# fnysalehi/Surface-Irradiance-Estimation-from-Neural-Radiance-Fields

Measured on AMD Instinct MI355X. Metric: Mrays/s @1080p NeRF inference (Lego snapshot); PSNR vs reference, higher is better.
Workload: dtype f16; 1 GPU; Lego-shaped synthetic scene (HashGrid L8 F4 T2^19 b=2.0, density MLP 32-64-16, rgb MLP 32-64-64-16, aabb_scale 1), 1920x1080 pinhole camera fov_x 0.6911 rad, 8 orbit azimuths, 1 spp, render_mode Shade, min_transmittance 0.01; frames_in_flight=2

## Files before the change

__graft_entry__.py:

```python
import importlib
import os
import sys

ROOT = os.path.dirname(os.path.abspath(__file__))
PKG = "surface-irradiance-estimation-from-neural-radiance-fields_amd"
if ROOT not in sys.path:
    sys.path.insert(0, ROOT)


def _pkg(sub):
    return importlib.import_module(PKG + "." + sub)


def build():
    lib = _pkg("build").build()
    _pkg("build").build(legacy=True)
    _pkg("build").build(nocache=True)
    _pkg("build").build(netsec_v1=True)
    _pkg("build").build_pyngp()
    _pkg("build").build_main()
    sys.path.insert(0, os.path.join(ROOT, "oracle"))
    import oracle as orc

    orc.build()
    native = _pkg("native")
    L = native.load_library()
    missing = [s for s in native.EXPORTS if not hasattr(L, s)]
    if missing:
        raise RuntimeError(f"libngp_hip.so lacks symbols: {missing}")
    print(f"built {lib}; {L.ngp_version().decode()}")


def smoke():
    import numpy as np

    sys.path.insert(0, os.path.join(ROOT, "oracle"))
    import oracle as orc

    native, synthetic, scene = _pkg("native"), _pkg("synthetic"), _pkg("scene")
    sc = synthetic.make_scene(aabb_scale=1, seed=7, log2_hashmap_size=15)
    ctx = native.Context(0)
    ctx.set_model(sc)
    w, h = 96, 54
    mat = scene.orbit_camera(45.0)
    focal = scene.focal_from_fov_x(w, 0.6911)
    img, depth = ctx.render(native.make_camera(mat, w, h, focal), native.make_opts(), want_depth=True)
    st = ctx.render_stats()
    o = orc.Oracle()
    bf, _ = o.density_grid_to_bitfield(np.asarray(sc["density_grid"], np.float16).astype(np.float32), sc["max_cascade"])
    sc["density_grid_bitfield"] = bf
    m = o.make_model(sc)
    fb, db, ost = o.render_nerf(m, o.make_camera(mat, w, h, focal))
    ref = o.tonemap(o.accumulate(fb.reshape(-1, 4), np.zeros((w * h, 4), np.float32), 0)).reshape(h, w, 4)
    err = float(np.quantile(np.abs(img - ref), 0.9995))
    mse = float(((np.clip(img[..., :3], 0, 1) - np.clip(ref[..., :3], 0, 1)) ** 2).mean())
    psnr = 99.0 if mse == 0 else -10.0 * np.log10(mse)
    print(f"smoke: {w}x{h} hit={st['n_rays_hit']} (oracle {ost['n_rays_hit']}) samples={st['n_samples']} (oracle {ost['n_samples']}) "
          f"q99.95|d|={err:.2e} psnr={psnr:.1f} dB kernel={st['kernel_ms']:.3f} ms")
    assert st["n_rays_hit"] > 0 and psnr > 45.0 and err < 2e-2, "HIP render does not match the oracle"
    o.release(m)
    fsc = synthetic.make_scene(aabb_scale=1, seed=7, cfg=scene.frequency_network_config())
    fsc["density_grid_bitfield"] = bf
    ctx.set_model(fsc)
    rng = np.random.default_rng(0)
    pos = rng.uniform(0, 1, (777, 3)).astype(np.float32)
    d01 = rng.uniform(0, 1, (777, 3)).astype(np.float32)
    got = ctx.network(pos, d01).astype(np.float32)
    fm = o.make_model(fsc)
    want = o.network(fm, pos, d01).astype(np.float32)
    o.release(fm)
    ferr = float(np.abs(got - want).max())
    print(f"smoke: frequency.json network, 777 samples, max |d logit| = {ferr:.2e}")
    assert np.isfinite(got).all() and ferr < 6e-2, "the frequency.json network does not match the oracle"
    ctx.close()


if __name__ == "__main__":
    build()
    if "--smoke" in sys.argv:
        smoke()
```

surface-irradiance-estimation-from-neural-radiance-fields_amd/build.py:

```python
import os
import subprocess
import sys

HERE = os.path.dirname(os.path.abspath(__file__))
CSRC = os.path.join(HERE, "csrc")
LIB = os.path.join(HERE, "libngp_hip.so")
SOURCES = ["nerf_kernels.hip", "wide_kernels.hip", "mesh_kernels.hip", "train_kernels.hip", "mc_kernels.hip", "ngp_api.cpp", "ngp_model.cpp", "ngp_snapshot.cpp", "ngp_dataset.cpp", "ngp_render.cpp", "ngp_mesh.cpp", "ngp_train.cpp", "ngp_multi.cpp", "ngp_mc.cpp"]
FLAGS = ["--offload-arch=gfx950", "-O3", "-std=c++17", "-fPIC", "-shared", "-ffp-contract=off", "-fno-slp-vectorize", "-fvisibility=hidden", "-Wall", "-Wno-unused-function"]


def hipcc():
    for c in (os.environ.get("HIPCC"), "/opt/rocm/bin/hipcc", "hipcc"):
        if c and (os.path.isabs(c) and os.path.exists(c) or not os.path.isabs(c)):
            return c
    raise RuntimeError("hipcc not found")


LIB_LEGACY = os.path.join(HERE, "libngp_hip_legacy.so")
LIB_CELLSTATS = os.path.join(HERE, "libngp_hip_cellstats.so")
LIB_NOCACHE = os.path.join(HERE, "libngp_hip_nocache.so")
LIB_NETSEC_V1 = os.path.join(HERE, "libngp_hip_netsec_v1.so")


def needs_build(lib=LIB):
    if not os.path.exists(lib):
        return True
    t = os.path.getmtime(lib)
    for f in os.listdir(CSRC):
        if os.path.getmtime(os.path.join(CSRC, f)) > t:
            return True
    inc = os.path.join(HERE, "..", "include", "ngp_hip.h")
    return os.path.getmtime(inc) > t


def build(force=False, verbose=False, legacy=False, nocache=False, cellstats=False, netsec_v1=False):
    if legacy + nocache + cellstats + netsec_v1 > 1:
        raise ValueError("one variant at a time")
    lib = LIB_LEGACY if legacy else LIB_NOCACHE if nocache else LIB_CELLSTATS if cellstats else LIB_NETSEC_V1 if netsec_v1 else LIB
    if not force and not needs_build(lib):
        return lib
    srcs = [os.path.join(CSRC, s) for s in SOURCES if os.path.exists(os.path.join(CSRC, s))]
    tmp = "%s.%d.tmp" % (lib, os.getpid())
    cmd = [hipcc()] + FLAGS + (["-DNGP_TCNN_LEGACY_ENCODE"] if legacy else []) + (["-DNGP_NO_CELL_CACHE"] if nocache else []) + (["-DNGP_EXPERIMENT_CELL_CACHE_STATS"] if cellstats else []) + (["-DNGP_NETSEC_V1"] if netsec_v1 else []) + os.environ.get("NGP_BUILD_DEFINES", "").split() + ["-o", tmp] + srcs + ["-lz"]
    if verbose:
        print(" ".join(cmd))
    r = subprocess.run(cmd, capture_output=True, text=True)
    if r.returncode != 0:
        sys.stderr.write(r.stdout + r.stderr)
        if os.path.exists(tmp):
            os.remove(tmp)
        raise RuntimeError("hipcc failed")
    os.replace(tmp, lib)
    return lib


def pyngp_path():
    import sysconfig

    return os.path.join(HERE, "pyngp" + sysconfig.get_config_var("EXT_SUFFIX"))


def build_pyngp(force=False, verbose=False):
    import pybind11
    import sysconfig

    out = pyngp_path()
    srcs = [os.path.join(CSRC, "pyngp.cpp"), os.path.join(CSRC, "testbed_shim.h"), os.path.join(HERE, "..", "include", "ngp_hip.h")]
    if not force and os.path.exists(out) and all(os.path.getmtime(out) >= os.path.getmtime(s) for s in srcs):
        return out
    build()
    cmd = ["g++", "-O2", "-std=c++17", "-shared", "-fPIC", "-fvisibility=hidden", "-I", sysconfig.get_paths()["include"], "-I", pybind11.get_include(),
           srcs[0], "-o", out + ".%d.tmp" % os.getpid(), "-L", HERE, "-lngp_hip", "-Wl,-rpath,$ORIGIN"]
    if verbose:
        print(" ".join(cmd))
    r = subprocess.run(cmd, capture_output=True, text=True)
    if r.returncode != 0:
        sys.stderr.write(r.stdout + r.stderr)
        raise RuntimeError("building pyngp failed")
    os.replace(out + ".%d.tmp" % os.getpid(), out)
    return out


def main_path():
    return os.path.join(HERE, "ngp_hip_main")


def build_main(force=False, verbose=False):
    out = main_path()
    srcs = [os.path.join(CSRC, "ngp_main.cpp"), os.path.join(CSRC, "testbed_shim.h"), os.path.join(CSRC, "minijson.h"), os.path.join(HERE, "..", "include", "ngp_hip.h")]
    if not force and os.path.exists(out) and all(os.path.getmtime(out) >= os.path.getmtime(s) for s in srcs):
        return out
    build()
    cmd = ["g++", "-O2", "-std=c++17", "-Wall", srcs[0], "-o", out + ".%d.tmp" % os.getpid(), "-L", HERE, "-lngp_hip", "-lz", "-Wl,-rpath,$ORIGIN"]
    if verbose:
        print(" ".join(cmd))
    r = subprocess.run(cmd, capture_output=True, text=True)
    if r.returncode != 0:
        sys.stderr.write(r.stdout + r.stderr)
        raise RuntimeError("building ngp_hip_main failed")
    os.replace(out + ".%d.tmp" % os.getpid(), out)
    return out


def import_pyngp():
    import importlib.util

    path = build_pyngp()
    spec = importlib.util.spec_from_file_location("pyngp", path)
    mod = importlib.util.module_from_spec(spec)
    spec.loader.exec_module(mod)
    return mod


if __name__ == "__main__":
    print(build(force="--force" in sys.argv, verbose=True))
    print(build_pyngp(force="--force" in sys.argv, verbose=True))
```

surface-irradiance-estimation-from-neural-radiance-fields_amd/csrc/nerf_device.h:

```cpp
#pragma once

#include "ngp_kernels.h"
#include "cell_cache.h"

namespace ngp {

typedef _Float16 half_t;
typedef _Float16 half8 __attribute__((ext_vector_type(8)));
typedef float floatx4 __attribute__((ext_vector_type(4)));

struct f3 {
	float x, y, z;
};

#define NGP_DEV __device__ __forceinline__

#ifdef NGP_CENSUS
#define NGP_SECTION(name) asm volatile("; SECTION " name)
#else
#define NGP_SECTION(name)
#endif

NGP_DEV f3 mk3(float x, float y, float z) { return f3{x, y, z}; }
NGP_DEV f3 add3(f3 a, f3 b) { return mk3(a.x + b.x, a.y + b.y, a.z + b.z); }
NGP_DEV f3 sub3(f3 a, f3 b) { return mk3(a.x - b.x, a.y - b.y, a.z - b.z); }
NGP_DEV f3 mul3(f3 a, f3 b) { return mk3(a.x * b.x, a.y * b.y, a.z * b.z); }
NGP_DEV f3 div3(f3 a, f3 b) { return mk3(a.x / b.x, a.y / b.y, a.z / b.z); }
NGP_DEV f3 scale3(f3 a, float s) { return mk3(a.x * s, a.y * s, a.z * s); }
NGP_DEV f3 adds3(f3 a, float s) { return mk3(a.x + s, a.y + s, a.z + s); }
NGP_DEV float dot3(f3 a, f3 b) { return (a.x * b.x + a.y * b.y) + a.z * b.z; }
NGP_DEV f3 normalize3(f3 a) {
	float len = __builtin_sqrtf(dot3(a, a));
	return mk3(a.x / len, a.y / len, a.z / len);
}
NGP_DEV f3 m3_mulv(const float* m, f3 v) {
	f3 r = mk3(m[0] * v.x, m[1] * v.x, m[2] * v.x);
	r = add3(r, mk3(m[3] * v.y, m[4] * v.y, m[5] * v.y));
	r = add3(r, mk3(m[6] * v.z, m[7] * v.z, m[8] * v.z));
	return r;
}

NGP_DEV uint32_t laine_karras_permutation(uint32_t x, uint32_t seed) {
	x += seed;
	x ^= x * 0x6c50b47cu;
	x ^= x * 0xb82f1e52u;
	x ^= x * 0xc7afe638u;
	x ^= x * 0x8d22f6e6u;
	return x;
}
NGP_DEV uint32_t nested_uniform_scramble_base2(uint32_t x, uint32_t seed) {
	x = __builtin_bitreverse32(x);
	x = laine_karras_permutation(x, seed);
	return __builtin_bitreverse32(x);
}
NGP_DEV uint32_t hash_combine(uint32_t seed, uint32_t v) { return seed ^ (v + (seed << 6) + (seed >> 2)); }
NGP_DEV float ld_random_val_dim0(uint32_t index, uint32_t seed) {
	index = nested_uniform_scramble_base2(index, seed);
	uint32_t x = nested_uniform_scramble_base2(__builtin_bitreverse32(index), hash_combine(seed, 0u));
	return (float)x * 2.3283064365386963e-10f;
}

NGP_DEV float stepsize() { return 1.73205080757f / (float)NERF_STEPS; }
NGP_DEV float max_cone_stepsize() { return stepsize() * (float)(1u << (NERF_CASCADES - 1)) * (float)NERF_STEPS / (float)NERF_GRIDSIZE; }

NGP_DEV float div_const(float x, float d, float rc) {
	float q0 = x * rc;
	float r = __builtin_fmaf(-q0, d, x);
	return __builtin_fmaf(r, rc, q0);
}
NGP_DEV float div_stepsize(float x) { return div_const(x, stepsize(), 1.0f / stepsize()); }
NGP_DEV float div_max_cone_stepsize(float x) { return div_const(x, max_cone_stepsize(), 1.0f / max_cone_stepsize()); }

struct Stepping {
	float cone_angle, log1p_c, a, b, at, bt;
	float to_scale, from_scale;
};
NGP_DEV Stepping make_stepping(float cone_angle) {
	Stepping s;
	s.cone_angle = cone_angle;
	s.log1p_c = s.a = s.b = s.at = s.bt = s.to_scale = s.from_scale = 0.0f;
	if (cone_angle <= 1e-5f) return s;
	s.log1p_c = logf(1.0f + cone_angle);
	s.a = (logf(stepsize()) - logf(s.log1p_c)) / s.log1p_c;
	s.b = (logf(max_cone_stepsize()) - logf(s.log1p_c)) / s.log1p_c;
	s.at = expf(s.a * s.log1p_c);
	s.bt = expf(s.b * s.log1p_c);
	s.to_scale = 0.6931471805599453f / s.log1p_c;
	s.from_scale = s.log1p_c * 1.4426950408889634f;
	return s;
}
NGP_DEV float to_stepping_space(float t, const Stepping& s) {
	if (s.cone_angle <= 1e-5f) return div_stepsize(t);
	if (t <= s.at) return div_stepsize(t - s.at) + s.a;
#ifdef NGP_PRECISE_STEPPING
	else if (t <= s.bt) return logf(t) / s.log1p_c;
#else
	else if (t <= s.bt) return __builtin_amdgcn_logf(t) * s.to_scale;
#endif
	else return div_max_cone_stepsize(t - s.bt) + s.b;
}
NGP_DEV float from_stepping_space(float n, const Stepping& s) {
	if (s.cone_angle <= 1e-5f) return n * stepsize();
	if (n <= s.a) return (n - s.a) * stepsize() + s.at;
#ifdef NGP_PRECISE_STEPPING
	else if (n <= s.b) return expf(n * s.log1p_c);
#else
	else if (n <= s.b) return __builtin_amdgcn_exp2f(n * s.from_scale);
#endif
	else return (n - s.b) * max_cone_stepsize() + s.bt;
}
NGP_DEV float advance_n_steps(float t, const Stepping& s, float n) { return from_stepping_space(to_stepping_space(t, s) + n, s); }
NGP_DEV float calc_dt(float t, const Stepping& s) { return advance_n_steps(t, s, 1.0f) - t; }
NGP_DEV float to_stepping_space(float t, float cone_angle) { return to_stepping_space(t, make_stepping(cone_angle)); }
NGP_DEV float from_stepping_space(float n, float cone_angle) { return from_stepping_space(n, make_stepping(cone_angle)); }
NGP_DEV float advance_n_steps(float t, float cone_angle, float n) { return advance_n_steps(t, make_stepping(cone_angle), n); }
NGP_DEV float calc_dt(float t, float cone_angle) { return calc_dt(t, make_stepping(cone_angle)); }
NGP_DEV float warp_dt(float dt) {
	const float max_stepsize = stepsize() * (float)(1u << (NERF_CASCADES - 1));
	return div_const(dt - stepsize(), max_stepsize - stepsize(), 1.0f / (max_stepsize - stepsize()));
}
NGP_DEV float unwarp_dt(float dt) {
	float max_stepsize = stepsize() * (float)(1u << (NERF_CASCADES - 1));
	return dt * (max_stepsize - stepsize()) + stepsize();
}

NGP_DEV uint32_t expand_bits(uint32_t v) {
	v = (v * 0x00010001u) & 0xFF0000FFu;
	v = (v * 0x00000101u) & 0x0F00F00Fu;
	v = (v * 0x00000011u) & 0xC30C30C3u;
	v = (v * 0x00000005u) & 0x49249249u;
	return v;
}
NGP_DEV uint32_t morton3D(uint32_t x, uint32_t y, uint32_t z) { return expand_bits(x) | (expand_bits(y) << 1) | (expand_bits(z) << 2); }
NGP_DEV uint32_t morton3D_invert(uint32_t x) {
	x = x & 0x49249249u;
	x = (x | (x >> 2)) & 0xc30c30c3u;
	x = (x | (x >> 4)) & 0x0f00f00fu;
	x = (x | (x >> 8)) & 0xff0000ffu;
	x = (x | (x >> 16)) & 0x0000ffffu;
	return x;
}

NGP_DEV bool density_grid_occupied_at(f3 pos, const uint8_t* __restrict__ bitfield, uint32_t mip) {
	float mip_scale = __builtin_ldexpf(1.0f, -(int)mip);
	pos = adds3(scale3(adds3(pos, -0.5f), mip_scale), 0.5f);
	int ix = (int)(pos.x * (float)NERF_GRIDSIZE);
	int iy = (int)(pos.y * (float)NERF_GRIDSIZE);
	int iz = (int)(pos.z * (float)NERF_GRIDSIZE);
	if (ix < 0 || ix >= (int)NERF_GRIDSIZE || iy < 0 || iy >= (int)NERF_GRIDSIZE || iz < 0 || iz >= (int)NERF_GRIDSIZE) return false;
	uint32_t idx = morton3D((uint32_t)ix, (uint32_t)iy, (uint32_t)iz);
	return (bitfield[idx / 8 + (NERF_GRID_N_CELLS / 8) * mip] & (1u << (idx % 8))) != 0;
}

NGP_DEV bool density_grid_occupied_at_lds(f3 pos, const uint8_t* __restrict__ bitfield, const uint32_t* s_coarse, uint32_t mip) {
	float mip_scale = __builtin_ldexpf(1.0f, -(int)mip);
	pos = adds3(scale3(adds3(pos, -0.5f), mip_scale), 0.5f);
	int ix = (int)(pos.x * (float)NERF_GRIDSIZE);
	int iy = (int)(pos.y * (float)NERF_GRIDSIZE);
	int iz = (int)(pos.z * (float)NERF_GRIDSIZE);
	if (ix < 0 || ix >= (int)NERF_GRIDSIZE || iy < 0 || iy >= (int)NERF_GRIDSIZE || iz < 0 || iz >= (int)NERF_GRIDSIZE) return false;
	uint32_t idx = morton3D((uint32_t)ix, (uint32_t)iy, (uint32_t)iz);
	uint32_t block = idx >> 6;
	if (!((s_coarse[mip * COARSE_WORDS_PER_MIP + (block >> 5)] >> (block & 31u)) & 1u)) return false;
	return (bitfield[idx / 8 + (NERF_GRID_N_CELLS / 8) * mip] & (1u << (idx % 8))) != 0;
}

struct OccBlockCache {
	uint32_t key;
	uint2 bits;
};

NGP_DEV uint32_t empty_block_size_at(f3 pos, const uint8_t* __restrict__ bitfield, const uint32_t* s_coarse, const uint32_t* s_coarse16, uint32_t mip,
                                     OccBlockCache& cache) {
	float mip_scale = __builtin_ldexpf(1.0f, -(int)mip);
	pos = adds3(scale3(adds3(pos, -0.5f), mip_scale), 0.5f);
	int ix = (int)(pos.x * (float)NERF_GRIDSIZE);
	int iy = (int)(pos.y * (float)NERF_GRIDSIZE);
	int iz = (int)(pos.z * (float)NERF_GRIDSIZE);
	if (ix < 0 || ix >= (int)NERF_GRIDSIZE || iy < 0 || iy >= (int)NERF_GRIDSIZE || iz < 0 || iz >= (int)NERF_GRIDSIZE) return 1u;
	uint32_t idx = morton3D((uint32_t)ix, (uint32_t)iy, (uint32_t)iz);
	uint32_t b16 = idx >> 12;
	if (!((s_coarse16[mip * 16u + (b16 >> 5)] >> (b16 & 31u)) & 1u)) return 16u;
	uint32_t b4 = idx >> 6;
	if (!((s_coarse[mip * COARSE_WORDS_PER_MIP + (b4 >> 5)] >> (b4 & 31u)) & 1u)) return 4u;
	const uint32_t key = (mip << 26) | b4;
	if (cache.key != key) {
		cache.bits = *(const uint2*)(bitfield + (size_t)b4 * 8 + (size_t)(NERF_GRID_N_CELLS / 8) * mip);
		cache.key = key;
	}
	const uint32_t word = (idx & 32u) ? cache.bits.y : cache.bits.x;
	return ((word >> (idx & 31u)) & 1u) ? 0u : 1u;
}

struct OccBlock {
	uint32_t key;
	uint2 bits;
};
NGP_DEV uint32_t occupancy_state_at(f3 pos, const uint8_t* __restrict__ bitfield, const uint32_t* s_coarse, const uint32_t* s_coarse16, uint32_t mip, OccBlock& cache,
                                    uint32_t lds_mips = NERF_CASCADES, const uint32_t* __restrict__ g_coarse = nullptr) {
	float mip_scale = __builtin_ldexpf(1.0f, -(int)mip);
	pos = adds3(scale3(adds3(pos, -0.5f), mip_scale), 0.5f);
	const int ix = (int)(pos.x * (float)NERF_GRIDSIZE);
	const int iy = (int)(pos.y * (float)NERF_GRIDSIZE);
	const int iz = (int)(pos.z * (float)NERF_GRIDSIZE);
	if (((uint32_t)ix | (uint32_t)iy | (uint32_t)iz) >= NERF_GRIDSIZE) return 1u;
	const uint32_t x = (uint32_t)ix, y = (uint32_t)iy, z = (uint32_t)iz;
	const uint32_t key = (x >> 2) | ((y >> 2) << 5) | ((z >> 2) << 10) | (mip << 15);
	if (cache.key != key) {
		const uint32_t b4 = morton3D(x >> 2, y >> 2, z >> 2), b16 = b4 >> 6;
		if (!((s_coarse16[mip * 16u + (b16 >> 5)] >> (b16 & 31u)) & 1u)) return 16u;
		const uint32_t cw = mip < lds_mips ? s_coarse[mip * COARSE_WORDS_PER_MIP + (b4 >> 5)] : g_coarse[mip * COARSE_WORDS_PER_MIP + (b4 >> 5)];
		if (!((cw >> (b4 & 31u)) & 1u)) return 4u;
		cache.bits = *(const uint2*)(bitfield + (size_t)b4 * 8 + (size_t)(NERF_GRID_N_CELLS / 8) * mip);
		cache.key = key;
	}
	const uint32_t bit = (x & 1u) | ((y & 1u) << 1) | ((z & 1u) << 2) | ((x & 2u) << 2) | ((y & 2u) << 3) | ((z & 2u) << 4);
	const uint32_t word = (bit & 32u) ? cache.bits.y : cache.bits.x;
	return ((word >> (bit & 31u)) & 1u) ? 0u : 1u;
}

NGP_DEV uint32_t empty_block_summary_at(f3 pos, const uint32_t* s_coarse, const uint32_t* s_coarse16, uint32_t mip, uint32_t lds_mips = NERF_CASCADES,
                                        const uint32_t* __restrict__ g_coarse = nullptr) {
	float mip_scale = __builtin_ldexpf(1.0f, -(int)mip);
	pos = adds3(scale3(adds3(pos, -0.5f), mip_scale), 0.5f);
	const int ix = (int)(pos.x * (float)(NERF_GRIDSIZE / 4)), iy = (int)(pos.y * (float)(NERF_GRIDSIZE / 4)), iz = (int)(pos.z * (float)(NERF_GRIDSIZE / 4));
	if (((uint32_t)ix | (uint32_t)iy | (uint32_t)iz) >= NERF_GRIDSIZE / 4 || pos.x < 0.0f || pos.y < 0.0f || pos.z < 0.0f) return 0u;
	const uint32_t b4 = morton3D((uint32_t)ix, (uint32_t)iy, (uint32_t)iz), b16 = b4 >> 6;
	if (!((s_coarse16[mip * 16u + (b16 >> 5)] >> (b16 & 31u)) & 1u)) return 16u;
	const uint32_t cw = mip < lds_mips ? s_coarse[mip * COARSE_WORDS_PER_MIP + (b4 >> 5)] : g_coarse[mip * COARSE_WORDS_PER_MIP + (b4 >> 5)];
	return ((cw >> (b4 & 31u)) & 1u) ? 0u : 4u;
}

NGP_DEV float distance_to_next_voxel(f3 pos, f3 dir, f3 idir, float res, float inv_res) {
	f3 p = scale3(adds3(pos, -0.5f), res);
	float tx = (__builtin_floorf(p.x + 0.5f + 0.5f * __builtin_copysignf(1.0f, dir.x)) - p.x) * idir.x;
	float ty = (__builtin_floorf(p.y + 0.5f + 0.5f * __builtin_copysignf(1.0f, dir.y)) - p.y) * idir.y;
	float tz = (__builtin_floorf(p.z + 0.5f + 0.5f * __builtin_copysignf(1.0f, dir.z)) - p.z) * idir.z;
	float t = fminf(fminf(tx, ty), tz);
	return fmaxf(t * inv_res, 0.0f);
}
NGP_DEV float advance_to_next_voxel(float t, const Stepping& s, f3 pos, f3 dir, f3 idir, uint32_t mip, uint32_t block = 1u) {
	const int shift = block == 16u ? 4 : (block == 4u ? 2 : 0);
	float res = __builtin_ldexpf((float)NERF_GRIDSIZE, -(int)mip - shift);
	float t_target = t + distance_to_next_voxel(pos, dir, idir, res, __builtin_ldexpf(1.0f / (float)NERF_GRIDSIZE, (int)mip + shift));
	t = to_stepping_space(t, s);
	t_target = to_stepping_space(t_target, s);
	return from_stepping_space(t + __builtin_ceilf(fmaxf(t_target - t, 0.5f)), s);
}
NGP_DEV float advance_to_next_voxel(float t, float cone_angle, f3 pos, f3 dir, f3 idir, uint32_t mip, uint32_t block = 1u) {
	return advance_to_next_voxel(t, make_stepping(cone_angle), pos, dir, idir, mip, block);
}
NGP_DEV float grid_cube_entry(f3 pos, f3 idir, float h) {
	const float lo = 0.5f - h, hi = 0.5f + h;
	float tx0 = (lo - pos.x) * idir.x, tx1 = (hi - pos.x) * idir.x;
	float ty0 = (lo - pos.y) * idir.y, ty1 = (hi - pos.y) * idir.y;
	float tz0 = (lo - pos.z) * idir.z, tz1 = (hi - pos.z) * idir.z;
	float tmin = fmaxf(fmaxf(fminf(tx0, tx1), fminf(ty0, ty1)), fminf(tz0, tz1));
	float tmax = fminf(fminf(fmaxf(tx0, tx1), fmaxf(ty0, ty1)), fmaxf(tz0, tz1));
	tmin = fmaxf(tmin, 0.0f);
	return tmax >= tmin ? tmin : -1.0f;
}
NGP_DEV float advance_by_distance(float t, const Stepping& s, float distance) {
	float t_target = t + distance;
	t = to_stepping_space(t, s);
	t_target = to_stepping_space(t_target, s);
	return from_stepping_space(t + __builtin_ceilf(fmaxf(t_target - t, 0.5f)), s);
}
NGP_DEV float advance_by_distance(float t, float cone_angle, float distance) { return advance_by_distance(t, make_stepping(cone_angle), distance); }
NGP_DEV uint32_t mip_from_pos(f3 pos, uint32_t max_cascade) {
	int exponent;
	float maxval = fmaxf(fmaxf(__builtin_fabsf(pos.x - 0.5f), __builtin_fabsf(pos.y - 0.5f)), __builtin_fabsf(pos.z - 0.5f));
	(void)__builtin_frexpf(maxval, &exponent);
	int v = exponent + 1;
	v = v < 0 ? 0 : v;
	v = v > (int)max_cascade ? (int)max_cascade : v;
	return (uint32_t)v;
}

NGP_DEV bool raabb_contains(const ModelParams& M, f3 p) {
	if (!M.r2l_identity) p = m3_mulv(M.r2l, p);
	return p.x >= M.raabb_min[0] && p.x <= M.raabb_max[0] && p.y >= M.raabb_min[1] && p.y <= M.raabb_max[1] && p.z >= M.raabb_min[2] && p.z <= M.raabb_max[2];
}

template <bool CAPPED>
NGP_DEV float skip_empty_space(float t, const ModelParams& M, f3 o, f3 d, f3 idir) {
	const float cone_angle = M.cone_angle;
	uint32_t i = 1;
	while (!CAPPED || i < 200) {
		f3 pos = add3(o, scale3(d, t));
		if (t >= MAX_DEPTH || !raabb_contains(M, pos)) return MAX_DEPTH;
		uint32_t mip = mip_from_pos(pos, NERF_CASCADES - 1);
		mip = mip > M.max_cascade ? M.max_cascade : mip;
		if (density_grid_occupied_at(pos, M.bitfield, mip)) return t;
		while (mip < M.max_cascade && !density_grid_occupied_at(pos, M.bitfield, mip + 1)) ++mip;
		t = advance_to_next_voxel(t, cone_angle, pos, d, idir, mip);
		++i;
	}
	return MAX_DEPTH;
}

NGP_DEV float aabb_ray_entry(const float* bmin, const float* bmax, f3 pos, f3 dir) {
	const float FMAX = 3.402823466e+38f;
	float tmin = (bmin[0] - pos.x) / dir.x;
	float tmax = (bmax[0] - pos.x) / dir.x;
	if (tmin > tmax) { float s = tmin; tmin = tmax; tmax = s; }
	float tymin = (bmin[1] - pos.y) / dir.y;
	float tymax = (bmax[1] - pos.y) / dir.y;
	if (tymin > tymax) { float s = tymin; tymin = tymax; tymax = s; }
	if (tmin > tymax || tymin > tmax) return FMAX;
	if (tymin > tmin) tmin = tymin;
	if (tymax < tmax) tmax = tymax;
	float tzmin = (bmin[2] - pos.z) / dir.z;
	float tzmax = (bmax[2] - pos.z) / dir.z;
	if (tzmin > tzmax) { float s = tzmin; tzmin = tzmax; tzmax = s; }
	if (tmin > tzmax || tzmin > tmax) return FMAX;
	if (tzmin > tmin) tmin = tzmin;
	return tmin;
}

struct RayState {
	f3 o, d;
	float t;
	uint32_t idx;
	uint32_t out;
	bool alive;
};

NGP_DEV void opencv_lens_distortion_delta(const float* q, float u, float v, float* du, float* dv) {
	const float k1 = q[0], k2 = q[1], p1 = q[2], p2 = q[3];
	const float u2 = u * u, uv = u * v, v2 = v * v, r2 = u2 + v2;
	const float radial = k1 * r2 + k2 * r2 * r2;
	*du = u * radial + 2.0f * p1 * uv + p2 * (r2 + 2.0f * u2);
	*dv = v * radial + 2.0f * p2 * uv + p1 * (r2 + 2.0f * v2);
}
NGP_DEV void opencv_fisheye_lens_distortion_delta(const float* q, float u, float v, float* du, float* dv) {
	const float k1 = q[0], k2 = q[1], k3 = q[2], k4 = q[3];
	const float r = __builtin_sqrtf(u * u + v * v);
	if (r > (float)2.220446049250313e-16) {
		const float theta = atanf(r);
		const float theta2 = theta * theta, theta4 = theta2 * theta2, theta6 = theta4 * theta2, theta8 = theta4 * theta4;
		const float thetad = theta * (1.0f + k1 * theta2 + k2 * theta4 + k3 * theta6 + k4 * theta8);
		*du = u * thetad / r - u;
		*dv = v * thetad / r - v;
	} else {
		*du = 0.0f;
		*dv = 0.0f;
	}
}
template <bool FISHEYE>
NGP_DEV void iterative_lens_undistortion(const float* q, float* u, float* v) {
	auto delta = [&](float a, float b, float* da, float* db) {
		if (FISHEYE) opencv_fisheye_lens_distortion_delta(q, a, b, da, db);
		else opencv_lens_distortion_delta(q, a, b, da, db);
	};
	const float x0 = *u, y0 = *v;
	float x = x0, y = y0;
	for (uint32_t i = 0; i < 100u; ++i) {
		const float step0 = fmaxf(1.1920929e-07f, __builtin_fabsf(1e-6f * x));
		const float step1 = fmaxf(1.1920929e-07f, __builtin_fabsf(1e-6f * y));
		float dx0, dx1, b0, b1, f0, f1, c0, c1, g0, g1;
		delta(x, y, &dx0, &dx1);
		delta(x - step0, y, &b0, &b1);
		delta(x + step0, y, &f0, &f1);
		delta(x, y - step1, &c0, &c1);
		delta(x, y + step1, &g0, &g1);
		const float j00 = 1.0f + (f0 - b0) / (2.0f * step0), j10 = (g0 - c0) / (2.0f * step1);
		const float j01 = (f1 - b1) / (2.0f * step0), j11 = 1.0f + (g1 - c1) / (2.0f * step1);
		const float rx = x + dx0 - x0, ry = y + dx1 - y0;
		const float det = j00 * j11 - j10 * j01;
		const float sx = (j11 * rx - j10 * ry) / det, sy = (-j01 * rx + j00 * ry) / det;
		x -= sx;
		y -= sy;
		if (sx * sx + sy * sy < 1e-10f) break;
	}
	*u = x;
	*v = y;
}
__device__ __attribute__((noinline)) void lens_direction_general(int lens_mode, const float* lens_params, float u, float v, float sx, float sy, float* out) {
	const float PI = 3.14159265358979323846f;
	f3 dir;
	if (lens_mode == 3) {
		float theta = (v - 0.5f) * PI, phi = (u - 0.5f) * PI * 2.0f;
// ... 107 lines not shown
	const float phi = atan2f(dy, dx);
	const float cyl_x = theta / PI, cyl_y = phi / (2.0f * PI) + 0.5f;
	const float fx = cyl_y * (float)(res_x - 1), fy = cyl_x * (float)(res_y - 1);
	const int tx = (int)fx, ty = (int)fy;
	const float wx = fx - (float)tx, wy = fy - (float)ty;
	auto read_val = [&](int px, int py) {
		if (px < 0) px += res_x;
		else if (px >= res_x) px -= res_x;
		py = py > res_y - 1 ? res_y - 1 : py;
		py = py < 0 ? 0 : py;
		return envmap[px + (size_t)py * res_x];
	};
	const float4 v00 = read_val(tx, ty), v10 = read_val(tx + 1, ty), v01 = read_val(tx, ty + 1), v11 = read_val(tx + 1, ty + 1);
	const float w00 = (1 - wx) * (1 - wy), w10 = wx * (1 - wy), w01 = (1 - wx) * wy, w11 = wx * wy;
	out4[0] = ((w00 * v00.x + w10 * v10.x) + w01 * v01.x) + w11 * v11.x;
	out4[1] = ((w00 * v00.y + w10 * v10.y) + w01 * v01.y) + w11 * v11.y;
	out4[2] = ((w00 * v00.z + w10 * v10.z) + w01 * v01.z) + w11 * v11.z;
	out4[3] = ((w00 * v00.w + w10 * v10.w) + w01 * v01.w) + w11 * v11.w;
}

template <bool PLAIN = false>
NGP_DEV void init_ray(const ModelParams& M, const CameraParams& C, uint32_t x, uint32_t y, RayState& r) {
	r.idx = x + (uint32_t)C.width * y;
	r.out = r.idx;
	float u = ((float)x + C.pixel_offset[0]) / (float)C.width;
	float v = ((float)y + C.pixel_offset[1]) / (float)C.height;
	f3 dir;
	if (PLAIN) dir = mk3((u - C.screen_center[0]) * (float)C.width / C.focal[0], (v - C.screen_center[1]) * (float)C.height / C.focal[1], 1.0f);
	else lens_direction(C, u, v, dir);
	f3 origin;
	if (PLAIN || !C.moving) {
		dir = m3_mulv(C.m, dir);
		origin = mk3(C.m[9], C.m[10], C.m[11]);
		if (!PLAIN && C.aperture_size != 0.0f) {
			float o3[3] = {origin.x, origin.y, origin.z}, d3[3] = {dir.x, dir.y, dir.z}, cm[6];
			for (int i = 0; i < 6; ++i) cm[i] = C.m[i];
			apply_aperture(cm, C.aperture_size, C.focus_z, C.spp, (uint32_t)(int)(u * (float)C.width) * 19349663u + (uint32_t)(int)(v * (float)C.height) * 96925573u, o3, d3);
			origin = mk3(o3[0], o3[1], o3[2]);
			dir = mk3(d3[0], d3[1], d3[2]);
		}
	} else {
		float cam[12], m0[12], m1[12], rs[4];
		for (int i = 0; i < 12; ++i) { m0[i] = C.m[i]; m1[i] = C.m1[i]; }
		for (int i = 0; i < 4; ++i) rs[i] = C.rolling_shutter[i];
		camera_at_pixel(m0, m1, rs, u, v, ld_random_val_dim0(C.spp, r.idx * 72239731u), cam);
		dir = m3_mulv(cam, dir);
		origin = mk3(cam[9], cam[10], cam[11]);
		if (C.aperture_size != 0.0f) {
			float o3[3] = {origin.x, origin.y, origin.z}, d3[3] = {dir.x, dir.y, dir.z};
			apply_aperture(cam, C.aperture_size, C.focus_z, C.spp, (uint32_t)(int)(u * (float)C.width) * 19349663u + (uint32_t)(int)(v * (float)C.height) * 96925573u, o3, d3);
			origin = mk3(o3[0], o3[1], o3[2]);
			dir = mk3(d3[0], d3[1], d3[2]);
		}
	}
	origin = add3(origin, scale3(dir, C.near_distance));
	r.o = origin;
	r.d = mk3(0.f, 0.f, 0.f);
	r.t = 0.f;
	r.alive = false;
	if (dir.x == 0.0f && dir.y == 0.0f && dir.z == 0.0f) return;
	dir = normalize3(dir);
	r.d = dir;
	float t = fmaxf(aabb_ray_entry(M.raabb_min, M.raabb_max, m3_mulv(M.r2l, origin), m3_mulv(M.r2l, dir)), 0.0f) + 1e-6f;
	if (!raabb_contains(M, add3(origin, scale3(dir, t)))) return;
	r.t = t;
	r.alive = true;
}

NGP_DEV void advance_pos(const ModelParams& M, const CameraParams& C, RayState& r) {
	if (!r.alive) return;
	f3 idir = mk3(1.0f / r.d.x, 1.0f / r.d.y, 1.0f / r.d.z);
	float t = advance_n_steps(r.t, M.cone_angle, ld_random_val_dim0(C.spp, r.idx * 786433u));
	t = skip_empty_space<false>(t, M, r.o, r.d, idir);
	if (t >= MAX_DEPTH) r.alive = false;
	else r.t = t;
}

struct CornerSet {
	uint32_t index[8];
};

struct CellPos {
	uint32_t gx, gy, gz;
	float wx, wy, wz;
};
NGP_DEV CellPos level_cell(const LevelInfo& L, float x, float y, float z) {
	float fx = __builtin_fmaf(L.scale, x, 0.5f), fy = __builtin_fmaf(L.scale, y, 0.5f), fz = __builtin_fmaf(L.scale, z, 0.5f);
	float flx = __builtin_floorf(fx), fly = __builtin_floorf(fy), flz = __builtin_floorf(fz);
	CellPos c;
	c.gx = (uint32_t)(int)flx; c.gy = (uint32_t)(int)fly; c.gz = (uint32_t)(int)flz;
	c.wx = fx - flx; c.wy = fy - fly; c.wz = fz - flz;
	return c;
}
NGP_DEV CellPos level_cell_in_cube(const LevelInfo& L, float x, float y, float z) {
	const float fx = __builtin_fmaf(L.scale, x, 0.5f), fy = __builtin_fmaf(L.scale, y, 0.5f), fz = __builtin_fmaf(L.scale, z, 0.5f);
	CellPos c;
	c.gx = (uint32_t)fx; c.gy = (uint32_t)fy; c.gz = (uint32_t)fz;
	c.wx = __builtin_amdgcn_fractf(fx); c.wy = __builtin_amdgcn_fractf(fy); c.wz = __builtin_amdgcn_fractf(fz);
	return c;
}
NGP_DEV void corner_weights(const CellPos& p, float* weight) {
	float wx0 = 1.0f - p.wx, wy0 = 1.0f - p.wy, wz0 = 1.0f - p.wz;
#pragma unroll
	for (int c = 0; c < 8; ++c) {
		int bx = c & 1, by = (c >> 1) & 1, bz = (c >> 2) & 1;
		weight[c] = ((bx ? p.wx : wx0) * (by ? p.wy : wy0)) * (bz ? p.wz : wz0);
	}
}
NGP_DEV bool level_in_xor_range(const LevelInfo& L, const CellPos& p) {
	uint32_t m = p.gx > p.gy ? p.gx : p.gy;
	m = m > p.gz ? m : p.gz;
	return m <= L.coord_max && !L.xor_disabled;
}
NGP_DEV bool unit_cube_in_xor_range(const LevelInfo* lv) {
	bool ok = true;
	for (int l = 0; l < N_LEVELS; ++l) ok = ok && !lv[l].xor_disabled && (uint32_t)__builtin_fmaf(lv[l].scale, 1.0f, 0.5f) <= lv[l].coord_max;
	return ok;
}
NGP_DEV bool in_unit_cube(float x, float y, float z) { return fminf(fminf(x, y), z) >= 0.0f && fmaxf(fmaxf(x, y), z) <= 1.0f; }

NGP_DEV void level_corners(const LevelInfo& L, const CellPos& p, CornerSet& cs) {
	uint32_t ix[2], iy[2], iz[2];
	if (L.hashed) {
		ix[0] = p.gx;               ix[1] = p.gx + 1u;
		iy[0] = p.gy * 2654435761u; iy[1] = (p.gy + 1u) * 2654435761u;
		iz[0] = p.gz * 805459861u;  iz[1] = (p.gz + 1u) * 805459861u;
	} else {
		uint32_t r2 = L.res * L.res;
		ix[0] = p.gx;         ix[1] = p.gx + 1u;
		iy[0] = p.gy * L.res; iy[1] = (p.gy + 1u) * L.res;
		iz[0] = p.gz * r2;    iz[1] = (p.gz + 1u) * r2;
	}
#pragma unroll
	for (int c = 0; c < 8; ++c) {
		int bx = c & 1, by = (c >> 1) & 1, bz = (c >> 2) & 1;
		uint32_t idx = L.hashed ? (ix[bx] ^ iy[by] ^ iz[bz]) : (ix[bx] + iy[by] + iz[bz]);
		idx = L.mask ? (idx & L.mask) : (idx % L.size);
		cs.index[c] = (L.offset + idx) * 8u;
	}
}

NGP_DEV void level_corners_xor(const LevelInfo& L, const CellPos& p, CornerSet& cs) {
	uint32_t ix[2], iy[2], iz[2];
	ix[0] = p.gx << 3;        ix[1] = ix[0] + 8u;
	iy[0] = p.gy * L.mul_y8;  iy[1] = iy[0] + L.mul_y8;
	iz[0] = p.gz * L.mul_z8;  iz[1] = iz[0] + L.mul_z8;
#pragma unroll
	for (int c = 0; c < 8; ++c) {
		int bx = c & 1, by = (c >> 1) & 1, bz = (c >> 2) & 1;
		cs.index[c] = ((ix[bx] ^ iy[by] ^ iz[bz]) & L.mask8) | L.base8;
	}
}

typedef unsigned int u32x2 __attribute__((ext_vector_type(2)));
typedef __amdgpu_buffer_rsrc_t GridRsrc;
NGP_DEV GridRsrc make_grid_rsrc(const void* table, uint32_t bytes) { return __builtin_amdgcn_make_buffer_rsrc(const_cast<void*>(table), (short)0, (int)bytes, 0x00020000); }
NGP_DEV uint2 gather8(GridRsrc r, uint32_t offset) {
	const u32x2 v = __builtin_amdgcn_raw_buffer_load_b64(r, (int)offset, 0, 0);
	return make_uint2(v.x, v.y);
}

typedef _Float16 half2_t __attribute__((ext_vector_type(2)));
NGP_DEV half_t to_half_rn(float v) {
	asm("" : "+v"(v));
	return (half_t)v;
}
struct FeatureAcc {
	half2_t f01, f23;
};
NGP_DEV float product_lo(float w, uint32_t packed) {
	float p;
	asm("v_fma_mix_f32 %0, %1, %2, 0 op_sel_hi:[0,1,0]" : "=v"(p) : "v"(w), "v"(packed));
	return p;
}
NGP_DEV float product_hi(float w, uint32_t packed) {
	float p;
	asm("v_fma_mix_f32 %0, %1, %2, 0 op_sel:[0,1,0] op_sel_hi:[0,1,0]" : "=v"(p) : "v"(w), "v"(packed));
	return p;
}
NGP_DEV void accumulate_corner(uint2 v, float w, FeatureAcc& r) {
#ifndef NGP_TCNN_LEGACY_ENCODE
	const half2_t wh = {(half_t)w, (half_t)w};
	const uint32_t wv = __builtin_bit_cast(uint32_t, wh);
	uint32_t a01 = __builtin_bit_cast(uint32_t, r.f01), a23 = __builtin_bit_cast(uint32_t, r.f23);
	asm("v_pk_fma_f16 %0, %1, %2, %0" : "+v"(a01) : "v"(wv), "v"(v.x));
	asm("v_pk_fma_f16 %0, %1, %2, %0" : "+v"(a23) : "v"(wv), "v"(v.y));
	r.f01 = __builtin_bit_cast(half2_t, a01);
	r.f23 = __builtin_bit_cast(half2_t, a23);
#else
	half2_t a, b;
	a[0] = (half_t)product_lo(w, v.x);
	a[1] = (half_t)product_hi(w, v.x);
	b[0] = (half_t)product_lo(w, v.y);
	b[1] = (half_t)product_hi(w, v.y);
	r.f01 = r.f01 + a;
	r.f23 = r.f23 + b;
#endif
}
NGP_DEV void accumulate_corner_pair(uint2 v0, uint2 v1, half2_t w01, FeatureAcc& r) {
	const uint32_t wv = __builtin_bit_cast(uint32_t, w01);
	uint32_t a01 = __builtin_bit_cast(uint32_t, r.f01), a23 = __builtin_bit_cast(uint32_t, r.f23);
	asm("v_pk_fma_f16 %0, %1, %2, %0 op_sel:[0,0,0] op_sel_hi:[0,1,1]" : "+v"(a01) : "v"(wv), "v"(v0.x));
	asm("v_pk_fma_f16 %0, %1, %2, %0 op_sel:[0,0,0] op_sel_hi:[0,1,1]" : "+v"(a23) : "v"(wv), "v"(v0.y));
	asm("v_pk_fma_f16 %0, %1, %2, %0 op_sel:[1,0,0] op_sel_hi:[1,1,1]" : "+v"(a01) : "v"(wv), "v"(v1.x));
	asm("v_pk_fma_f16 %0, %1, %2, %0 op_sel:[1,0,0] op_sel_hi:[1,1,1]" : "+v"(a23) : "v"(wv), "v"(v1.y));
	r.f01 = __builtin_bit_cast(half2_t, a01);
	r.f23 = __builtin_bit_cast(half2_t, a23);
}
NGP_DEV void store_features(const FeatureAcc& lo, const FeatureAcc& hi, half8& out) {
	out[0] = lo.f01[0]; out[1] = lo.f01[1]; out[2] = lo.f23[0]; out[3] = lo.f23[1];
	out[4] = hi.f01[0]; out[5] = hi.f01[1]; out[6] = hi.f23[0]; out[7] = hi.f23[1];
}

struct EncodeInFlight {
	uint2 v[16];
	float wx[2], wy[2], wz[2];
	uint32_t cell;
};
NGP_DEV void encode_issue(GridRsrc grid, GridRsrc xgrid, const LevelInfo* lv, int h, float x, float y, float z, EncodeInFlight& e) {
	const LevelInfo& L0 = lv[h];
	const LevelInfo& L1 = lv[h + 4];
	const CellPos p0 = level_cell(L0, x, y, z), p1 = level_cell(L1, x, y, z);
	CornerSet c0, c1;
	if (__all((int)level_in_xor_range(L0, p0) & (int)level_in_xor_range(L1, p1))) {
		level_corners_xor(L0, p0, c0);
		level_corners_xor(L1, p1, c1);
#pragma unroll
		for (int c = 0; c < 8; ++c) e.v[c] = gather8(xgrid, c0.index[c]);
#pragma unroll
		for (int c = 0; c < 8; ++c) e.v[8 + c] = gather8(xgrid, c1.index[c]);
#if defined(NGP_EXPERIMENT_EXTRA_GATHERS)
#pragma unroll
		for (int c = 0; c < NGP_EXPERIMENT_EXTRA_GATHERS; ++c) {
			const uint2 d = gather8(xgrid, c & 1 ? c1.index[c & 7] : c0.index[c & 7]);
			asm volatile("" ::"v"(d.x), "v"(d.y));
		}
#endif
	} else {
		level_corners(L0, p0, c0);
		level_corners(L1, p1, c1);
#pragma unroll
		for (int c = 0; c < 8; ++c) e.v[c] = gather8(grid, c0.index[c]);
#pragma unroll
		for (int c = 0; c < 8; ++c) e.v[8 + c] = gather8(grid, c1.index[c]);
	}
	e.wx[0] = p0.wx; e.wy[0] = p0.wy; e.wz[0] = p0.wz;
	e.wx[1] = p1.wx; e.wy[1] = p1.wy; e.wz[1] = p1.wz;
}
NGP_DEV half8 encode_finish(const EncodeInFlight& e) {
	NGP_SECTION("encode_finish");
	FeatureAcc acc[2] = {{{0, 0}, {0, 0}}, {{0, 0}, {0, 0}}};
#pragma unroll
	for (int l = 0; l < 2; ++l) {
		CellPos p;
		p.gx = p.gy = p.gz = 0;
		p.wx = e.wx[l]; p.wy = e.wy[l]; p.wz = e.wz[l];
		float w[8];
		corner_weights(p, w);
#if defined(NGP_TCNN_LEGACY_ENCODE) || defined(NGP_NETSEC_V1)
#pragma unroll
		for (int c = 0; c < 8; ++c) accumulate_corner(e.v[8 * l + c], w[c], acc[l]);
#else
#pragma unroll
		for (int c = 0; c < 8; c += 2) {
			const half2_t w01 = {to_half_rn(w[c]), to_half_rn(w[c + 1])};
			accumulate_corner_pair(e.v[8 * l + c], e.v[8 * l + c + 1], w01, acc[l]);
		}
#endif
	}
	half8 out;
	store_features(acc[0], acc[1], out);
	NGP_SECTION("network");
	return out;
}
constexpr int CELL_CACHE_SETS = 8;
struct CellCache {
	uint4 line[CELL_CACHE_LEVELS][CELL_CACHE_SETS][4];
	uint32_t tag[CELL_CACHE_LEVELS][CELL_CACHE_SETS];
};
NGP_DEV void cell_cache_clear(CellCache* caches, int n_waves, int thread, int n_threads) {
	for (int i = thread; i < n_waves * CELL_CACHE_LEVELS * CELL_CACHE_SETS; i += n_threads)
		caches[i / (CELL_CACHE_LEVELS * CELL_CACHE_SETS)].tag[i / CELL_CACHE_SETS % CELL_CACHE_LEVELS][i % CELL_CACHE_SETS] = CELL_TAG_NONE;
}
NGP_DEV void encode_issue_cached(GridRsrc grid, GridRsrc xgrid, const LevelInfo* lv, int h, float x, float y, float z, EncodeInFlight& e, CellCache& cc, bool in_cube) {
	NGP_SECTION("issue.cells");
	const LevelInfo& L0 = lv[h];
	const LevelInfo& L1 = lv[h + 4];
#ifdef NGP_NETSEC_V1
	CellPos p0 = level_cell(L0, x, y, z), p1 = level_cell(L1, x, y, z);
	in_cube = __all((int)level_in_xor_range(L0, p0) & (int)level_in_xor_range(L1, p1));
#else
	CellPos p0, p1;
#endif
	CornerSet c0, c1;
	e.cell = CELL_TAG_NONE;
	if (in_cube) {
#ifndef NGP_NETSEC_V1
		p0 = level_cell_in_cube(L0, x, y, z);
		p1 = level_cell_in_cube(L1, x, y, z);
#endif
		NGP_SECTION("issue.fine");
		level_corners_xor(L1, p1, c1);
#pragma unroll
		for (int c = 0; c < 8; ++c) e.v[8 + c] = gather8(xgrid, c1.index[c]);
		NGP_SECTION("issue.tag_lines");
		const bool cacheable = cell_cacheable(p0.gx, p0.gy, p0.gz);
		const uint32_t tag = cell_tag(p0.gx, p0.gy, p0.gz), set = cell_set(tag, CELL_CACHE_SETS);
		const bool hit = __hip_atomic_load(&cc.tag[h][set], __ATOMIC_RELAXED, __HIP_MEMORY_SCOPE_WAVEFRONT) == tag && cacheable;
#pragma unroll
		for (int q = 0; q < 4; ++q) {
			const uint4 d = cc.line[h][set][q];
			e.v[2 * q] = make_uint2(d.x, d.y);
			e.v[2 * q + 1] = make_uint2(d.z, d.w);
// ... 397 lines not shown
```

surface-irradiance-estimation-from-neural-radiance-fields_amd/csrc/nerf_kernels.hip:

```cpp
#include "render_common.h"
#include "pcg32.h"

namespace ngp {

constexpr int BLOCK = 256;

#if defined(NGP_NO_CELL_CACHE) || defined(NGP_EXPERIMENT_CELL_CACHE_STATS)
constexpr bool CELL_CACHE_BUILT = false;
#else
constexpr bool CELL_CACHE_BUILT = true;
#endif
struct FusedGeneric {
	static constexpr bool probe = false, unit = false, outside = true, plain = false, normals = false, cell_cache = false;
	static constexpr int prof = 0, mips = (int)NERF_CASCADES, rgb_mid = 1;
};
struct FusedUnit : FusedGeneric { static constexpr bool unit = true, cell_cache = CELL_CACHE_BUILT; static constexpr int mips = 1; };
struct FusedUnitPlain : FusedUnit { static constexpr bool plain = true; };
struct FusedC5 : FusedGeneric { static constexpr bool outside = false; static constexpr int mips = 4; };
struct FusedC5Plain : FusedC5 { static constexpr bool plain = true; };
struct FusedMid0 : FusedGeneric { static constexpr int rgb_mid = 0; };
struct FusedMid2 : FusedGeneric { static constexpr int rgb_mid = 2; };
struct FusedLinRgb : FusedGeneric { static constexpr int rgb_mid = -1; };
struct FusedLin : FusedGeneric { static constexpr int rgb_mid = -2; };
struct FusedNormals : FusedGeneric { static constexpr bool normals = true; };
struct FusedProf : FusedGeneric { static constexpr int prof = 1; };
struct FusedUnitPlainProf : FusedUnitPlain { static constexpr int prof = 1; };
struct FusedUnitPlainProf2 : FusedUnitPlain { static constexpr int prof = 2; };
struct FusedProbe : FusedGeneric { static constexpr bool probe = true; };

template <class V>
NGP_DEV void fused_body(const ModelParams& M, const CameraParams& C, const FrameParams& F, const ProbeParams& P) {
	constexpr bool PROBE = V::probe, UNIT = V::unit, OUTSIDE = V::outside, PLAIN = V::plain, NORMALS = V::normals, CELL_CACHE = V::cell_cache;
	constexpr int PROF = V::prof, MIPS = V::mips, RGB_MID = V::rgb_mid;
	const uint32_t max_cascade = UNIT ? 0u : M.max_cascade;
	const float cone_angle = UNIT ? 0.0f : M.cone_angle;
	const Stepping stepping = make_stepping(cone_angle);
	__shared__ uint4 s_w[n_frags_for(RGB_MID) * 64];
	__shared__ LevelInfo s_lv[N_LEVELS];
	__shared__ uint32_t s_coarse[MIPS * COARSE_WORDS_PER_MIP];
	__shared__ uint32_t s_coarse16[(UNIT ? 1 : (int)NERF_CASCADES) * 16];
	__shared__ uint2 s_sh[BLOCK * 4];
	constexpr int SLOTS = 64;
	__shared__ float4 s_samp[BLOCK / 64 * SLOTS];
	__shared__ uint2 s_res[BLOCK / 64 * SLOTS];
	__shared__ float4 s_nrm[NORMALS ? BLOCK / 64 * SLOTS : 1];
	__shared__ CellCache s_cells[CELL_CACHE ? BLOCK / 64 : 1];
#ifdef NGP_EXPERIMENT_CELL_CACHE_STATS
	__shared__ uint32_t s_cst[BLOCK / 64][CELL_CACHE_LEVELS][4 + 8 + 16];
	for (int i = threadIdx.x; i < BLOCK / 64 * CELL_CACHE_LEVELS * 28; i += BLOCK) (&s_cst[0][0][0])[i] = CELL_TAG_NONE;
	unsigned long long cst_n = 0, cst_hit[3] = {0, 0, 0};
#endif
	__shared__ uint32_t s_xstate, s_xcount, s_active;
	constexpr uint32_t XRAYS = 16;
	__shared__ float s_xray[XRAYS * 16];
	if (threadIdx.x == 0) {
		s_xstate = 0u;
		s_xcount = 0u;
		s_active = BLOCK / 64;
	}
	unsigned long long t_entry = 0, rt_entry = 0;
	if (PROF) { t_entry = stamp(); rt_entry = realtime(); }
	for (int i = threadIdx.x; i < n_frags_for(RGB_MID) * 64; i += BLOCK) s_w[i] = M.wfrags[i];
	if (threadIdx.x < N_LEVELS) s_lv[threadIdx.x] = M.levels[threadIdx.x];
	for (uint32_t i = threadIdx.x; i < (max_cascade + 1 < (uint32_t)MIPS ? max_cascade + 1 : (uint32_t)MIPS) * COARSE_WORDS_PER_MIP; i += BLOCK) s_coarse[i] = M.coarse[i];
	if (threadIdx.x < (UNIT ? 1 : (int)NERF_CASCADES) * 16) s_coarse16[threadIdx.x] = M.coarse[NERF_CASCADES * COARSE_WORDS_PER_MIP + threadIdx.x];
	if (CELL_CACHE) cell_cache_clear(s_cells, BLOCK / 64, threadIdx.x, BLOCK);
	__syncthreads();

	const int lane = threadIdx.x & 63;
	const int c = lane & 15;
	if (lane == 0 && (threadIdx.x >> 6) == 0) atomicMax(&F.results[4], ~realtime());
	const GridRsrc t_grid = make_grid_rsrc(M.grid, M.grid_bytes), t_xgrid = make_grid_rsrc(M.xgrid, M.xgrid_bytes);
	const bool cube_in_xor_range = CELL_CACHE && unit_cube_in_xor_range(M.levels);
	(void)cube_in_xor_range;
	const float* cam_last = (!PLAIN && C.moving) ? C.m1 : C.m;
	const f3 cam_fwd = mk3(cam_last[6], cam_last[7], cam_last[8]);
	const f3 bg_linear = (PROBE || !F.direct) ? mk3(0.f, 0.f, 0.f)
	                     : F.color_space == 1 ? mk3(F.background[0], F.background[1], F.background[2])
	                                          : mk3(srgb_to_linear(F.background[0]), srgb_to_linear(F.background[1]), srgb_to_linear(F.background[2]));
	const float4 empty_pixel = (!PROBE && F.direct) ? tonemap_pixel(F, bg_linear, 0.f, 0.f, 0.f, 0.f) : make_float4(0.f, 0.f, 0.f, 0.f);
	const f3 cam_pos = mk3(cam_last[9], cam_last[10], cam_last[11]);
	const f3 amin = mk3(M.aabb_min[0], M.aabb_min[1], M.aabb_min[2]);
	const f3 adiag = mk3(M.aabb_diag[0], M.aabb_diag[1], M.aabb_diag[2]);

	RayState ray;
	ray.alive = false;
	ray.o = ray.d = mk3(0.f, 0.f, 0.f);
	ray.t = 0.f;
	ray.idx = 0;
	ray.out = 0;
	f3 idir = mk3(0.f, 0.f, 0.f);
	Accum acc = {0.f, 0.f, 0.f, 0.f, 0.f, 0.f};
	uint32_t step = 1;
	uint32_t skip_i = 1;
	float t_max = 0.f;
	bool counted = false;
	uint32_t n_pend = 0, sl_lo = 0, sl_hi = 0;
	bool left_box = false;
	uint32_t n_slots = 0;
	const int wave_base = threadIdx.x & ~63;
	OccBlock occ_cache;
	occ_cache.key = 0xffffffffu;
	occ_cache.bits = make_uint2(0u, 0u);
	bool finished = false;
	bool idle = false;
	const uint32_t my_wave = threadIdx.x >> 6;

	bool exhausted = false;
	uint32_t qsel = (uint32_t)__builtin_amdgcn_s_getreg(20 | (0 << 6) | (3 << 11)) & 7u;
	int stall = 0;
	uint32_t n_alive_init = 0, n_hit = 0, n_samples = 0;
	unsigned long long p_skip[3] = {0, 0, 0};
	unsigned long long pt[4] = {0, 0, 0, 0}, p_iters = 0, p_passes = 0, p_rounds = 0, p_lane_steps = 0, t0 = 0, t1 = 0;

	unsigned long long rt_start = 0;
	if (PROF && F.prof) {
		rt_start = realtime();
		if (lane == 0) atomicMax(&F.prof[8], ~rt_start);
	}
	int tr_slot = -1;
	uint32_t tr_it = 0, tr_info0 = 0, tr_info1 = 0, tr_march = 0;
	uint32_t tr_net[7] = {0, 0, 0, 0, 0, 0, 0};
	unsigned long long tr_t[5] = {0, 0, 0, 0, 0};
	auto trace_emit = [&](int upto) {
		if (!PROF || tr_slot < 0) return;
		if (tr_it < F.trace_cap_iters && lane == 0) {
			uint32_t* r = F.trace + 16 + F.trace_cap_waves * 16u + ((size_t)tr_slot * F.trace_cap_iters + tr_it) * 16u;
			r[0] = (uint32_t)tr_t[0];
			for (int k = 1; k < 5; ++k) r[k] = (uint32_t)(tr_t[k <= upto ? k : upto] - tr_t[0]);
			r[5] = tr_info0;
			r[6] = tr_info1;
			r[7] = tr_march;
			for (int k = 0; k < 7; ++k) r[8 + k] = upto >= 3 ? tr_net[k] : 0u;
		}
		++tr_it;
	};
	for (;;) {
		if (PROF) { t0 = stamp(); tr_t[0] = t0; tr_info0 = tr_info1 = tr_march = 0; for (int k = 0; k < 7; ++k) tr_net[k] = 0; }
		unsigned long long dead_mask = __ballot(!ray.alive);
		int n_dead = __popcll(dead_mask);
		if ((exhausted || n_dead >= F.tune[0]) && __any(finished)) {
			bool hit = false;
			if (finished) {
				hit = shade_ray<PROBE, PLAIN, NORMALS>(F, P, bg_linear, ray.out, acc, step - 1u, ray.d);
				finished = false;
			}
			n_hit += (uint32_t)__popcll(__ballot(hit));
			if (PROF) tr_info1 |= 4u << 24;
		}
		if (!exhausted && n_dead >= (F.tune[0] > 16 ? F.tune[0] : 16)) {
			const uint32_t want = (uint32_t)n_dead >> 4, n_strips = F.n_local_tiles * 4u;
			uint32_t first = 0, limit = n_strips;
			if (!PROBE && F.xqueue) {
				for (int tries = 0; tries < 8; ++tries) {
					const uint32_t lo = (uint32_t)(((unsigned long long)n_strips * qsel) >> 3), hi = (uint32_t)(((unsigned long long)n_strips * (qsel + 1u)) >> 3);
					uint32_t off = 0;
					if (lane == 0) off = atomicAdd(F.xqueue + qsel, want);
					off = __builtin_amdgcn_readfirstlane(off);
					first = lo + off;
					limit = hi;
					if (off < hi - lo) break;
					first = limit = n_strips;
					qsel = (qsel + 1u) & 7u;
				}
			} else {
				if (lane == 0) first = atomicAdd(F.queue, want);
				first = __builtin_amdgcn_readfirstlane(first);
			}
			if (first >= limit) {
				exhausted = true;
			} else {
				const uint32_t got = limit - first < want ? limit - first : want;
				if (PROF && F.trace && tr_slot == -1) {
					uint32_t n = 0;
					if (lane == 0) n = atomicAdd(F.trace, 1u);
					n = __builtin_amdgcn_readfirstlane(n);
					tr_slot = (n % F.trace_stride == 0u && n / F.trace_stride < F.trace_cap_waves) ? (int)(n / F.trace_stride) : -2;
					if (tr_slot >= 0 && lane == 0) {
						uint32_t* hd = F.trace + 16 + (size_t)tr_slot * 16u;
						hd[0] = (uint32_t)__builtin_amdgcn_s_getreg(4 | (0 << 6) | (31 << 11));
						hd[1] = (uint32_t)__builtin_amdgcn_s_getreg(20 | (0 << 6) | (3 << 11)) & 7u;
						hd[2] = blockIdx.x;
						hd[3] = threadIdx.x >> 6;
						hd[5] = (uint32_t)rt_entry; hd[6] = (uint32_t)(rt_entry >> 32);
						hd[9] = (uint32_t)t_entry; hd[10] = (uint32_t)tr_t[0];
						hd[11] = n;
					}
				}
				if (PROF) tr_info1 |= 8u << 24;
				const uint32_t r = lanes_below(dead_mask);
				const uint32_t strip = first + (r >> 4);
				const bool take = !ray.alive && r < got * 16u;
				const uint32_t tile_local = strip >> 2, s4 = strip & 3u, i16 = r & 15u;
				const uint32_t slot = ((s4 >> 1) * 4u + (i16 >> 2)) * 8u + (s4 & 1u) * 4u + (i16 & 3u);
				const uint32_t tile = F.shard_index + F.shard_count * tile_local;
				bool fresh = false;
				if (PROBE) {
					uint32_t q = tile * 64u + slot;
					if (take && q < P.n_rays) {
						init_probe_ray(P, q, ray, t_max);
						fresh = ray.alive;
					}
				} else if (take) {
					uint32_t x = (tile % F.tiles_x) * 8u + (slot & 7u);
					uint32_t y = (tile / F.tiles_x) * 8u + (slot >> 3);
					if (x < (uint32_t)C.width && y < (uint32_t)C.height) {
						init_ray<PLAIN>(M, C, x, y, ray);
						if (F.packed) ray.out = tile_local * 64u + slot;
						if (PLAIN || !F.envmap) {
							if (F.direct) {
								F.frame_buffer[ray.out] = empty_pixel;
								F.depth_buffer[ray.out] = MAX_DEPTH;
							} else if (F.depth_buffer[ray.out] < 0.01f) {
								F.depth_buffer[ray.out] = MAX_DEPTH;
							}
						} else {
							const bool valid = ray.d.x != 0.0f || ray.d.y != 0.0f || ray.d.z != 0.0f;
							float env[4] = {0.f, 0.f, 0.f, 0.f};
							if (valid) {
								float d3[3] = {ray.d.x, ray.d.y, ray.d.z};
								read_envmap(F.envmap, F.env_w, F.env_h, d3, env);
							}
							if (F.direct) {
								F.frame_buffer[ray.out] = valid ? tonemap_pixel(F, bg_linear, env[0], env[1], env[2], env[3]) : empty_pixel;
								F.depth_buffer[ray.out] = MAX_DEPTH;
							} else {
								if (valid) F.frame_buffer[ray.out] = make_float4(env[0], env[1], env[2], env[3]);
								if (F.depth_buffer[ray.out] < 0.01f) F.depth_buffer[ray.out] = MAX_DEPTH;
							}
						}
						if (ray.alive) {
							ray.t = advance_n_steps(ray.t, stepping, ld_random_val_dim0(C.spp, ray.idx * 786433u));
							fresh = true;
						}
					}
				}
				if (fresh) {
					{
						union { half_t h[16]; uint2 u[4]; } sh;
						sh4_all((ray.d.x + 1.0f) * 0.5f, (ray.d.y + 1.0f) * 0.5f, (ray.d.z + 1.0f) * 0.5f, sh.h);
#pragma unroll
						for (int q = 0; q < 4; ++q) s_sh[threadIdx.x * 4 + q] = sh.u[q];
					}
					idir = mk3(1.0f / ray.d.x, 1.0f / ray.d.y, 1.0f / ray.d.z);
					acc = Accum{0.f, 0.f, 0.f, 0.f, 0.f, 0.f};
					step = 1;
					skip_i = 1;
					counted = PROBE;
				}
				if (PROBE) n_alive_init += (uint32_t)__popcll(__ballot(fresh));
			}
		}

		if (!PROBE && F.tune[7] && n_slots == 0u) {
			const uint32_t st = __hip_atomic_load(&s_xstate, __ATOMIC_RELAXED, __HIP_MEMORY_SCOPE_WORKGROUP);
			const unsigned long long live_mask = __ballot(ray.alive);
			if ((st & 0xf00u) == 0x100u && __popcll(live_mask) >= 16) {
				const uint32_t to = st & 0xffu;
				uint32_t won = 0;
				if (lane == 0) won = atomicCAS(&s_xstate, st, 0x200u | to) == st ? 1u : 0u;
				won = __builtin_amdgcn_readfirstlane(won);
				if (won) {
					const uint32_t rank = lanes_below(live_mask);
					if (ray.alive && (rank & 1u) && (rank >> 1) < XRAYS) {
						const uint32_t k = rank >> 1;
						float* x = s_xray + k * 16u;
						x[0] = ray.o.x; x[1] = ray.o.y; x[2] = ray.o.z;
						x[3] = ray.d.x; x[4] = ray.d.y; x[5] = ray.d.z;
						x[6] = ray.t;
						x[7] = __uint_as_float(ray.out);
						x[8] = acc.r; x[9] = acc.g; x[10] = acc.b; x[11] = acc.a; x[12] = acc.depth; x[13] = acc.max_weight;
						x[14] = __uint_as_float(step | (counted ? 0x80000000u : 0u));
						x[15] = __uint_as_float(ray.idx);
#pragma unroll
						for (int q = 0; q < 4; ++q) s_sh[(to * 64u + k) * 4u + q] = s_sh[threadIdx.x * 4 + q];
						ray.alive = false;
					}
					if (lane == 0) {
						atomicAdd(&s_active, 1u);
						const uint32_t n_out = (uint32_t)__popcll(live_mask) >> 1;
						s_xcount = n_out < XRAYS ? n_out : XRAYS;
						__hip_atomic_store(&s_xstate, 0x300u | to, __ATOMIC_RELEASE, __HIP_MEMORY_SCOPE_WORKGROUP);
					}
				}
			}
		}
		if (PROF) { t1 = stamp(); pt[0] += t1 - t0; t0 = t1; tr_t[1] = t1; }
		const int n_live = __popcll(__ballot(ray.alive));
		const int k_fit = n_live <= 8 ? 8 : (n_live <= 10 ? 6 : (n_live <= 12 ? 5 : (n_live <= 16 ? 4 : (n_live <= 21 ? 3 : 2))));
		const int k_max = PROBE ? 1 : (n_live > SLOTS / 2 ? F.tune[4] : (k_fit < F.tune[5] ? k_fit : F.tune[5]));
		const int max_it = F.tune[1] > k_max ? F.tune[1] : k_max;
		bool blocked = false;
		for (int k = 0; k < max_it; ++k) {
			NGP_SECTION("march");
			const bool marching = ray.alive && !left_box && !blocked && (int)n_pend < k_max;
			if (!__any(marching) || n_slots >= (uint32_t)SLOTS) break;
			if (PROF) { const uint32_t nm = (uint32_t)__popcll(__ballot(marching)); ++p_rounds; p_lane_steps += (unsigned long long)nm; tr_march += 1u + (nm << 8); }
			const f3 pos = add3(ray.o, scale3(ray.d, ray.t));
			bool out = ray.t >= MAX_DEPTH || !raabb_contains(M, pos);
			if (PROBE && skip_i >= 200) out = true;
			if (PROBE && ray.t >= t_max) out = true;
			const bool inside = marching && !out;
			uint32_t mip = 0, empty = 1u;
			if (inside) {
				if (!UNIT) {
					mip = mip_from_pos(pos, NERF_CASCADES - 1);
					mip = mip > max_cascade ? max_cascade : mip;
				}
				empty = occupancy_state_at(pos, M.bitfield, s_coarse, s_coarse16, mip, occ_cache, MIPS, M.coarse);
			}
			const bool emit = inside && empty == 0u;
			const bool skip = inside && empty != 0u;
			float e_dt = 0.f;
			f3 e_w = mk3(0.f, 0.f, 0.f);
			if (emit) {
				e_dt = calc_dt(ray.t, stepping);
				e_w = sub3(pos, amin);
				if (M.diag_pow2) e_w = mul3(e_w, mk3(M.aabb_inv_diag[0], M.aabb_inv_diag[1], M.aabb_inv_diag[2]));
				else e_w = div3(e_w, adiag);
			}
			bool ends = marching && out;
			if (skip) {
				if (!UNIT) {
					if (PROBE || !F.tune[6]) {
						while (mip < max_cascade) {
							uint32_t e = occupancy_state_at(pos, M.bitfield, s_coarse, s_coarse16, mip + 1, occ_cache, MIPS, M.coarse);
							if (e == 0u) break;
							++mip;
							empty = e;
						}
					} else {
						uint32_t best_mip = mip, best_empty = empty;
						for (uint32_t m = mip + 1u; m <= max_cascade; ++m) {
							const uint32_t e = empty_block_summary_at(pos, s_coarse, s_coarse16, m, MIPS, M.coarse);
							if (e == 0u) break;
							if ((e << m) >= (best_empty << best_mip)) { best_mip = m; best_empty = e; }
						}
						mip = best_mip;
						empty = best_empty;
					}
				}
				if (PROF) p_skip[empty == 16u ? 2 : (empty == 4u ? 1 : 0)] += 1ull;
				const float grid_half = 0.5f * (float)(1u << max_cascade);
				const bool outside = OUTSIDE && !PROBE && empty == 1u && mip == max_cascade &&
				                     fmaxf(fmaxf(__builtin_fabsf(pos.x - 0.5f), __builtin_fabsf(pos.y - 0.5f)), __builtin_fabsf(pos.z - 0.5f)) > grid_half;
				const float to_grid = outside ? grid_cube_entry(pos, idir, grid_half) : 0.0f;
				if (outside && to_grid < 0.0f) {
					ends = true;
				} else if (outside && to_grid > 0.0f) {
					ray.t = advance_by_distance(ray.t, stepping, to_grid);
				} else {
					ray.t = advance_to_next_voxel(ray.t, stepping, pos, ray.d, idir, mip, (PROBE || !F.tune[6]) ? 1u : empty);
				}
				++skip_i;
			}
			if (ends) {
				if (n_pend == 0) {
					ray.alive = false;
					finished = true;
				} else {
					left_box = true;
				}
			}
			const unsigned long long emit_mask = __ballot(emit);
			if (emit_mask) {
				const uint32_t slot = n_slots + lanes_below(emit_mask);
				bool newly_counted = false;
				if (emit) {
					newly_counted = !counted;
					counted = true;
					if (slot < (uint32_t)SLOTS) {
						s_samp[wave_base + slot] = make_float4(e_w.x, e_w.y, e_w.z, warp_dt(e_dt));
						s_res[wave_base + slot].x = (uint32_t)lane;
						if (n_pend < 4u) sl_lo |= slot << (8u * n_pend);
						else sl_hi |= slot << (8u * (n_pend - 4u));
						++n_pend;
						ray.t = ray.t + e_dt;
						skip_i = 1;
					} else {
						blocked = true;
					}
				}
				n_alive_init += (uint32_t)__popcll(__ballot(newly_counted));
				n_slots += (uint32_t)__popcll(emit_mask);
				n_slots = n_slots > (uint32_t)SLOTS ? (uint32_t)SLOTS : n_slots;
			}
		}
		NGP_SECTION("other");
		const bool can_march = __any(ray.alive && !left_box && !blocked && (int)n_pend < k_max);
		if (PROF) {
			t1 = stamp(); pt[1] += t1 - t0; t0 = t1; ++p_iters; tr_t[2] = t1;
			tr_info0 = n_slots | ((uint32_t)stall << 24);
			tr_info1 |= (uint32_t)__popcll(__ballot(ray.alive)) | ((uint32_t)__popcll(__ballot(ray.alive && !left_box && n_pend == 0)) << 8) | ((uint32_t)k_max << 16) |
			            ((exhausted ? 1u : 0u) << 24);
		}
		if (n_slots == 0) {
			trace_emit(2);
			if (exhausted && !__any(ray.alive) && !__any(finished)) {
				if (PROBE || !F.tune[7]) break;
				if (!idle) {
					idle = true;
					if (lane == 0) atomicSub(&s_active, 1u);
				}
				bool got = false;
				for (;;) {
					uint32_t st = 0, act = 0;
					if (lane == 0) {
						st = __hip_atomic_load(&s_xstate, __ATOMIC_ACQUIRE, __HIP_MEMORY_SCOPE_WORKGROUP);
						act = __hip_atomic_load(&s_active, __ATOMIC_RELAXED, __HIP_MEMORY_SCOPE_WORKGROUP);
					}
					st = __builtin_amdgcn_readfirstlane(st);
					act = __builtin_amdgcn_readfirstlane(act);
					if (st == (0x300u | my_wave)) {
						got = true;
						break;
					}
					if (act == 0u) break;
					if (st == 0u && lane == 0) atomicCAS(&s_xstate, 0u, 0x100u | my_wave);
					__builtin_amdgcn_s_sleep(32);
				}
				if (!got) break;
				const uint32_t n_in = s_xcount;
				if ((uint32_t)lane < n_in) {
					const float* x = s_xray + (uint32_t)lane * 16u;
					ray.o = mk3(x[0], x[1], x[2]);
					ray.d = mk3(x[3], x[4], x[5]);
					ray.t = x[6];
					ray.out = __float_as_uint(x[7]);
					acc = Accum{x[8], x[9], x[10], x[11], x[12], x[13]};
					const uint32_t sw = __float_as_uint(x[14]);
					step = sw & 0x7fffffffu;
					counted = (sw >> 31) != 0u;
					ray.idx = __float_as_uint(x[15]);
					idir = mk3(1.0f / ray.d.x, 1.0f / ray.d.y, 1.0f / ray.d.z);
					ray.alive = true;
					finished = false;
					left_box = false;
					skip_i = 1;
					n_pend = 0;
					sl_lo = sl_hi = 0;
					occ_cache.key = 0xffffffffu;
				}
				idle = false;
				if (lane == 0) __hip_atomic_store(&s_xstate, 0u, __ATOMIC_RELEASE, __HIP_MEMORY_SCOPE_WORKGROUP);
			}
			continue;
		}
		if ((int)n_slots < F.tune[2] && can_march && stall < F.tune[3]) {
			++stall;
			trace_emit(2);
			continue;
		}
		stall = 0;

		NGP_SECTION("network");
		const int n_pass = (int)((n_slots + 15u) >> 4);
		const int hq = lane >> 4;
		auto sample_of = [&](int p, float& sx, float& sy, float& sz, Sh4& shq) {
			NGP_SECTION("sample_of");
			const float4 a = s_samp[wave_base + 16 * p + c];
			const uint32_t owner = s_res[wave_base + 16 * p + c].x;
			sx = a.x; sy = a.y; sz = a.z;
			union { uint2 u; half_t h[4]; } cv;
#ifdef NGP_NETSEC_V1
			cv.u = s_sh[(wave_base + (int)owner) * 4 + hq];
#else
			cv.u = s_sh[(wave_base + (int)(owner & 63u)) * 4 + hq];
#endif
#pragma unroll
			for (int j = 0; j < 4; ++j) shq.v[j] = cv.h[j];
			NGP_SECTION("network");
		};
		auto deliver = [&](int p, const MlpOut& mo) {
			NGP_SECTION("deliver");
			union { half_t h[4]; uint2 u; } o;
			o.h[0] = mo.rgb[0]; o.h[1] = mo.rgb[1]; o.h[2] = mo.rgb[2]; o.h[3] = mo.sigma;
			if (lane < 16) s_res[wave_base + 16 * p + lane] = o.u;
			NGP_SECTION("network");
		};
		int p = 0;
		if (NORMALS) {
			for (; p < n_pass; ++p) {
				float ax, ay, az;
				Sh4 sha;
				sample_of(p, ax, ay, az, sha);
				EncodeInFlight e;
				encode_issue(t_grid, t_xgrid, s_lv, hq, ax, ay, az, e);
				const half8 enc = encode_finish(e);
				DensityGrad dg = density_gradient_pass(s_w, M.wfrags, lane, e, enc, s_lv[hq].scale, s_lv[hq + 4].scale, M.density_linear != 0);
#pragma unroll
				for (int k = 0; k < 3; ++k) {
					dg.g[k] += __shfl_xor(dg.g[k], 16, 64);
					dg.g[k] += __shfl_xor(dg.g[k], 32, 64);
				}
				if (lane < 16) s_nrm[wave_base + 16 * p + lane] = make_float4(dg.g[0] * (1.0f / 128.0f), dg.g[1] * (1.0f / 128.0f), dg.g[2] * (1.0f / 128.0f), (float)dg.sigma);
			}
		}
		bool round_in_cube = true;
#ifndef NGP_NETSEC_V1
		if constexpr (CELL_CACHE) {
			NGP_SECTION("round_range");
			const float4 a = s_samp[wave_base + lane];
			round_in_cube = cube_in_xor_range && !__any((uint32_t)lane < n_slots && !in_unit_cube(a.x, a.y, a.z));
			NGP_SECTION("network");
		}
#endif
		auto issue = [&](float sx, float sy, float sz, EncodeInFlight& e) {
			if constexpr (CELL_CACHE) encode_issue_cached(t_grid, t_xgrid, s_lv, hq, sx, sy, sz, e, s_cells[my_wave], round_in_cube);
			else encode_issue(t_grid, t_xgrid, s_lv, hq, sx, sy, sz, e);
#ifdef NGP_EXPERIMENT_CELL_CACHE_STATS
			const CellPos p = level_cell(s_lv[hq], sx, sy, sz);
			e.cell = CELL_TAG_NONE;
			if (level_in_xor_range(s_lv[hq], p) && cell_cacheable(p.gx, p.gy, p.gz)) {
				const uint32_t tag = cell_tag(p.gx, p.gy, p.gz);
				e.cell = tag;
				++cst_n;
				for (int k = 0; k < 3; ++k) {
					const bool hit = s_cst[my_wave][hq][(4 << k) - 4 + cell_set(tag, 4u << k)] == tag;
					cst_hit[k] += hit ? 1u : 0u;
					e.cell |= hit ? 0u : 1u << (24 + k);
				}
			}
#endif
		};
		auto keep = [&](const EncodeInFlight& e) {
			if constexpr (CELL_CACHE) cell_cache_fill(s_cells[my_wave], hq, e);
#ifdef NGP_EXPERIMENT_CELL_CACHE_STATS
			if (e.cell != CELL_TAG_NONE)
				for (int k = 0; k < 3; ++k)
					if (e.cell >> (24 + k) & 1u) s_cst[my_wave][hq][(4 << k) - 4 + cell_set(e.cell & 0xFFFFFFu, 4u << k)] = e.cell & 0xFFFFFFu;
#endif
		};
		unsigned long long u0 = 0, u1 = 0;
		auto lap = [&](int k, bool drain_gathers) {
			if (drain_gathers) asm volatile("s_waitcnt vmcnt(0)" ::: "memory");
			else if (k == 5) asm volatile("s_waitcnt lgkmcnt(0)" ::: "memory");
			u1 = stamp();
			tr_net[k] += (uint32_t)(u1 - u0);
			u0 = u1;
		};
		if (PROF >= 2) u0 = stamp();
		for (; p + 1 < n_pass; p += 2) {
			float ax, ay, az, bx, by, bz;
			Sh4 sha, shb;
			sample_of(p, ax, ay, az, sha);
			sample_of(p + 1, bx, by, bz, shb);
			EncodeInFlight ea, eb;
			issue(ax, ay, az, ea);
			issue(bx, by, bz, eb);
			if (PROF >= 2) { lap(0, false); if (CELL_CACHE) lap(5, false); lap(1, true); }
			half8 enca = encode_finish(ea);
			half8 encb = encode_finish(eb);
			if (PROF >= 2) lap(2, false);
			keep(ea);
			keep(eb);
			if (PROF >= 2 && CELL_CACHE) lap(6, false);
#ifdef NGP_NETSEC_V1
			MlpOut moa = mlp_pass<RGB_MID>(s_w, lane, enca, sha);
			MlpOut mob = mlp_pass<RGB_MID>(s_w, lane, encb, shb);
#else
			MlpOut moa, mob;
			mlp_pass2<RGB_MID>(s_w, lane, enca, sha, encb, shb, moa, mob);
#endif
			if (PROF >= 2) lap(3, false);
			deliver(p, moa);
			deliver(p + 1, mob);
			if (PROF >= 2) lap(4, false);
		}
		if (p < n_pass) {
			float ax, ay, az;
			Sh4 sha;
			sample_of(p, ax, ay, az, sha);
			EncodeInFlight e1;
			issue(ax, ay, az, e1);
			if (PROF >= 2) { lap(0, false); if (CELL_CACHE) lap(5, false); lap(1, true); }
			half8 enc = encode_finish(e1);
			if (PROF >= 2) lap(2, false);
			keep(e1);
			if (PROF >= 2 && CELL_CACHE) lap(6, false);
			MlpOut mo = mlp_pass<RGB_MID>(s_w, lane, enc, sha);
			if (PROF >= 2) lap(3, false);
			deliver(p, mo);
			if (PROF >= 2) lap(4, false);
		}

		if (PROF) { t1 = stamp(); pt[2] += t1 - t0; t0 = t1; p_passes += (unsigned long long)n_pass; tr_t[3] = t1; tr_info0 |= (n_slots << 8) | ((uint32_t)n_pass << 16); }
		for (uint32_t k = 0;; ++k) {
			NGP_SECTION("composite");
			const bool have = k < n_pend && ray.alive;
			if (!__any(have)) break;
			if (have) {
				const uint32_t slot = ((k < 4u ? sl_lo >> (8u * k) : sl_hi >> (8u * (k - 4u))) & 0xffu);
				const float4 a = s_samp[wave_base + slot];
				union { uint2 u; half_t h[4]; } o;
				o.u = s_res[wave_base + slot];
				float gx = 0.f, gy = 0.f, gz = 0.f;
				if (NORMALS) {
					const float4 g = s_nrm[wave_base + slot];
					gx = g.x; gy = g.y; gz = g.z;
					o.h[3] = (half_t)g.w;
				}
				const f3 pos = add3(amin, mul3(mk3(a.x, a.y, a.z), adiag));
				const float sdepth = PROBE ? dot3(ray.d, sub3(pos, ray.o))
				                          : dot3(cam_fwd, sub3(pos, cam_pos));
				float T = 1.0f - acc.a;
				float dt = unwarp_dt(a.w);
				float alpha = 1.0f - fast_exp(-network_to_density((float)o.h[3], M.density_act) * dt);
				float weight = alpha * T;
				float cr = network_to_rgb((float)o.h[0], M.rgb_act), cg = network_to_rgb((float)o.h[1], M.rgb_act), cb = network_to_rgb((float)o.h[2], M.rgb_act);
				if (!PROBE && F.render_mode > 1) {
					if (NORMALS) {
						const float dd = network_to_density_derivative((float)o.h[3], M.density_act);
						const f3 nrm = normalize3(mk3(-dd * gx, -dd * gy, -dd * gz));
						cr = nrm.x; cg = nrm.y; cb = nrm.z;
					} else if (F.render_mode == 2) {
						cr = cg = cb = alpha;
					} else if (F.render_mode == 3) {
						cr = (pos.x - 0.5f) / 2.0f + 0.5f; cg = (pos.y - 0.5f) / 2.0f + 0.5f; cb = (pos.z - 0.5f) / 2.0f + 0.5f;
					} else {
						cr = cg = cb = dot3(cam_fwd, sub3(pos, ray.o)) * F.depth_scale;
					}
				}
				acc.r += cr * weight;
				acc.g += cg * weight;
				acc.b += cb * weight;
				acc.a += weight;
				if (weight > acc.max_weight) {
					acc.max_weight = weight;
					acc.depth = sdepth;
				}
				++step;
				if (acc.a > (1.0f - F.min_transmittance)) {
					acc.r /= acc.a; acc.g /= acc.a; acc.b /= acc.a; acc.a /= acc.a;
					ray.alive = false;
					finished = true;
				} else if (step >= MARCH_ITER) {
					ray.alive = false;
				}
			}
			n_samples += (uint32_t)__popcll(__ballot(have));
		}
		NGP_SECTION("other");
		if (left_box && ray.alive) {
			ray.alive = false;
			finished = true;
		}
		left_box = false;
		n_pend = 0;
		sl_lo = sl_hi = 0;
		n_slots = 0;
		if (PROF) { t1 = stamp(); pt[3] += t1 - t0; tr_t[4] = t1; trace_emit(4); }
	}
	if (PROF) {
		for (int k = 0; k < 3; ++k)
			for (int off = 32; off > 0; off >>= 1) p_skip[k] += __shfl_down(p_skip[k], off, 64);
	}
	if (PROF && tr_slot >= 0 && lane == 0) {
		uint32_t* hd = F.trace + 16 + (size_t)tr_slot * 16u;
		const unsigned long long rt_end = realtime(), t_end = stamp();
		hd[4] = tr_it;
		hd[7] = (uint32_t)rt_end; hd[8] = (uint32_t)(rt_end >> 32);
		hd[12] = (uint32_t)t_end;
		hd[13] = n_samples;
	}
	if (PROF && lane == 0 && F.prof) {
		for (int k = 0; k < 3; ++k) atomicAdd(&F.prof[12 + k], p_skip[k]);
		for (int k = 0; k < 4; ++k) atomicAdd(&F.prof[k], pt[k]);
		atomicAdd(&F.prof[4], p_iters);
		atomicAdd(&F.prof[5], p_passes);
		atomicAdd(&F.prof[6], p_rounds);
		atomicAdd(&F.prof[7], p_lane_steps);
		unsigned long long t_end = realtime(), t_first = ~F.prof[8];
		atomicMax(&F.prof[9], t_end);
		unsigned long long bucket = (t_end - t_first) / 10000ull;
		if (bucket > 47ull) bucket = 47ull;
		atomicAdd(&F.prof[16 + bucket], 1ull);
	}

#ifdef NGP_EXPERIMENT_CELL_CACHE_STATS
	if (F.prof) {
		for (int off = 8; off > 0; off >>= 1) {
			cst_n += __shfl_xor(cst_n, off, 64);
			for (int k = 0; k < 3; ++k) cst_hit[k] += __shfl_xor(cst_hit[k], off, 64);
		}
		if (c == 0) {
			atomicAdd(&F.prof[64 + 4 * (lane >> 4)], cst_n);
			for (int k = 0; k < 3; ++k) atomicAdd(&F.prof[64 + 4 * (lane >> 4) + 1 + k], cst_hit[k]);
		}
	}
#endif
	finish_launch(F, lane, n_alive_init, n_hit, n_samples);
}

#define NGP_FUSED_KERNEL(NAME, WAVES, V) \
	__global__ __launch_bounds__(BLOCK, WAVES) void NAME(const ModelParams M, const CameraParams C, const FrameParams F) { \
		ProbeParams P{}; \
		fused_body<V>(M, C, F, P); \
	}
NGP_FUSED_KERNEL(render_nerf_fused, 2, FusedGeneric)
NGP_FUSED_KERNEL(render_nerf_fused_unit, 3, FusedUnit)
NGP_FUSED_KERNEL(render_nerf_fused_unit_plain, 3, FusedUnitPlain)
NGP_FUSED_KERNEL(render_nerf_fused_c5_plain, 3, FusedC5Plain)
NGP_FUSED_KERNEL(render_nerf_fused_c5, 3, FusedC5)
NGP_FUSED_KERNEL(render_nerf_fused_mid0, 2, FusedMid0)
NGP_FUSED_KERNEL(render_nerf_fused_mid2, 2, FusedMid2)
NGP_FUSED_KERNEL(render_nerf_fused_lin_rgb, 2, FusedLinRgb)
NGP_FUSED_KERNEL(render_nerf_fused_lin, 2, FusedLin)
NGP_FUSED_KERNEL(render_nerf_fused_normals, 2, FusedNormals)
NGP_FUSED_KERNEL(render_nerf_fused_prof, 2, FusedProf)
NGP_FUSED_KERNEL(render_nerf_fused_unit_plain_prof, 3, FusedUnitPlainProf)
NGP_FUSED_KERNEL(render_nerf_fused_unit_plain_prof2, 3, FusedUnitPlainProf2)

__global__ __launch_bounds__(BLOCK, 2) void trace_probe_fused(const ModelParams M, const FrameParams F, const ProbeParams P) {
	CameraParams C{};
	fused_body<FusedProbe>(M, C, F, P);
}

__global__ void probe_reduce_kernel(const ProbeParams P, float4* __restrict__ envmap) {
	uint32_t texel = blockIdx.x * blockDim.x + threadIdx.x;
	const uint32_t per_probe = P.n_theta * P.n_phi, n_probes = P.mode == 3 ? P.grid_x * P.grid_y : 1u;
	if (texel >= per_probe * n_probes) return;
	if (P.mode == 3) {
		envmap[texel] = P.ray_rgba[texel];
		return;
	}
	const uint32_t no = P.mode == 2 ? P.n_origin : 1u;
	uint32_t i = texel % P.n_theta, j = texel / P.n_theta;
	float4 acc = make_float4(0.f, 0.f, 0.f, 0.f);
	for (uint32_t pr = 0; pr < no; ++pr) {
		for (uint32_t tr = 0; tr < no; ++tr) {
			float4 v = P.ray_rgba[(i * no + tr) + P.n_theta * no * (j * no + pr)];
			acc.x += v.x; acc.y += v.y; acc.z += v.z; acc.w += v.w;
		}
	}
	float inv = 1.0f / (float)(no * no);
	envmap[texel] = make_float4(acc.x * inv, acc.y * inv, acc.z * inv, acc.w * inv);
}

struct IrradianceQuery {
	uint32_t n_theta, n_phi;
	const float4* envmap;
	uint32_t n;
	const float* normals;
	int32_t outward;
	float origin[3], center[3];
	uint32_t grid_x, grid_y;
	float shell_radius;
	float4* out;
};
__global__ void irradiance_kernel(const IrradianceQuery Q) {
	__shared__ double s[3][256];
	const uint32_t q = blockIdx.x;
	if (q >= Q.n) return;
	const uint32_t texels = Q.n_theta * Q.n_phi;
	const uint32_t probe = Q.normals ? 0u : q / texels;
	f3 nrm;
	if (!Q.normals) nrm = cylindrical_to_dir_nerf((float)((q % texels) % Q.n_theta) / (float)Q.n_theta, (float)((q % texels) / Q.n_theta) / (float)Q.n_phi);
	else nrm = mk3(Q.normals[3 * (size_t)q], Q.normals[3 * (size_t)q + 1], Q.normals[3 * (size_t)q + 2]);
	float frame[9] = {1, 0, 0, 0, 1, 0, 0, 0, 1};
	if (Q.outward) {
		const f3 origin = Q.outward == 3 ? probe_grid_origin(Q.center, Q.grid_x, Q.grid_y, Q.shell_radius, probe) : mk3(Q.origin[0], Q.origin[1], Q.origin[2]);
		local_frame(normalize3(origin), frame);
	}
	const float4* envmap = Q.envmap + (size_t)texels * probe;
	double a0 = 0, a1 = 0, a2 = 0;
	for (uint32_t t = threadIdx.x; t < texels; t += blockDim.x) {
		f3 w = cylindrical_to_dir_nerf((float)(t % Q.n_theta) / (float)Q.n_theta, (float)(t / Q.n_theta) / (float)Q.n_phi);
		if (Q.outward) w = scale3(normalize3(m3_mulv(frame, w)), -1.0f);
		float c = dot3(nrm, w);
		if (c > 0.0f) {
			float4 L = envmap[t];
			a0 += (double)(L.x * c); a1 += (double)(L.y * c); a2 += (double)(L.z * c);
		}
	}
	s[0][threadIdx.x] = a0; s[1][threadIdx.x] = a1; s[2][threadIdx.x] = a2;
	__syncthreads();
	for (int off = 128; off > 0; off >>= 1) {
		if ((int)threadIdx.x < off) {
			s[0][threadIdx.x] += s[0][threadIdx.x + off];
			s[1][threadIdx.x] += s[1][threadIdx.x + off];
			s[2][threadIdx.x] += s[2][threadIdx.x + off];
		}
		__syncthreads();
	}
	if (threadIdx.x == 0) {
		const double d_omega = 4.0 * 3.14159265358979323846 / ((double)Q.n_theta * (double)Q.n_phi);
		Q.out[q] = make_float4((float)(s[0][0] * d_omega), (float)(s[1][0] * d_omega), (float)(s[2][0] * d_omega), 0.f);
	}
}

__global__ __launch_bounds__(BLOCK) void grid_encode_kernel(const ModelParams M, uint32_t n, const float* __restrict__ pos01, uint16_t* __restrict__ out) {
	__shared__ LevelInfo s_lv[N_LEVELS];
// ... 62 lines not shown
	for (int p = 0; p < 4; ++p) {
		const uint32_t s = wave * 64u + 16u * p + c;
		const uint32_t sc = s < n ? s : n - 1;
		EncodeInFlight e;
		encode_issue(t_grid, t_xgrid, s_lv, hq, pos01[3 * sc], pos01[3 * sc + 1], pos01[3 * sc + 2], e);
		const half8 enc = encode_finish(e);
		DensityGrad dg = density_gradient_pass(s_w, M.wfrags, lane, e, enc, s_lv[hq].scale, s_lv[hq + 4].scale, M.density_linear != 0);
#pragma unroll
		for (int k = 0; k < 3; ++k) {
			dg.g[k] += __shfl_xor(dg.g[k], 16, 64);
			dg.g[k] += __shfl_xor(dg.g[k], 32, 64);
		}
		if (s < n && lane < 16) {
#pragma unroll
			for (int k = 0; k < 3; ++k) out[(size_t)s * 3 + k] = dg.g[k] * (1.0f / 128.0f);
		}
	}
}

template <bool DLIN>
__global__ __launch_bounds__(BLOCK) void density_grid_samples_kernel(const ModelParams M, uint32_t n_samples, Pcg32 rng, uint32_t step, uint32_t n_cascades,
                                                                     float thresh, const float* __restrict__ grid_in, float* __restrict__ grid_tmp) {
	__shared__ uint4 s_w[N_FRAGS * 64];
	__shared__ LevelInfo s_lv[N_LEVELS];
	for (int i = threadIdx.x; i < N_FRAGS * 64; i += BLOCK) s_w[i] = M.wfrags[i];
	if (threadIdx.x < N_LEVELS) s_lv[threadIdx.x] = M.levels[threadIdx.x];
	__syncthreads();
	const int lane = threadIdx.x & 63, c = lane & 15;
	const GridRsrc t_grid = make_grid_rsrc(M.grid, M.grid_bytes), t_xgrid = make_grid_rsrc(M.xgrid, M.xgrid_bytes);
	const uint32_t t = blockIdx.x * BLOCK + threadIdx.x;
	constexpr uint32_t A = 56924617u, C = 96925573u;
	constexpr uint32_t AINV = []() { uint32_t x = A; for (int k = 0; k < 5; ++k) x *= 2u - A * x; return x; }();
	static_assert(A * AINV == 1u, "modular inverse");
	const uint32_t n_whole = n_samples & ~(NERF_GRID_N_CELLS - 1u);
	const uint32_t i = t < n_whole ? ((t & ~(NERF_GRID_N_CELLS - 1u)) | ((((t & (NERF_GRID_N_CELLS - 1u)) - C) * AINV - step * n_samples) & (NERF_GRID_N_CELLS - 1u))) : t;
	const bool valid = i < n_samples;
	rng.advance((uint64_t)i * 4u);
	const uint32_t level = (uint32_t)(rng.next_float() * (float)n_cascades) % n_cascades;
	uint32_t idx = 0;
	for (uint32_t j = 0; j < 10; ++j) {
		idx = ((i + step * n_samples) * 56924617u + j * 19349663u + 96925573u) % NERF_GRID_N_CELLS;
		idx += level * NERF_GRID_N_CELLS;
		if (!valid || grid_in[idx] > thresh) break;
	}
	const uint32_t pos_idx = idx % NERF_GRID_N_CELLS;
	const float x = (float)morton3D_invert(pos_idx >> 0), y = (float)morton3D_invert(pos_idx >> 1), z = (float)morton3D_invert(pos_idx >> 2);
	const float rx = rng.next_float(), ry = rng.next_float(), rz = rng.next_float();
	const float scale = __builtin_ldexpf(1.0f, (int)level);
	f3 pos = mk3(((x + rx) / (float)NERF_GRIDSIZE - 0.5f) * scale + 0.5f, ((y + ry) / (float)NERF_GRIDSIZE - 0.5f) * scale + 0.5f,
	             ((z + rz) / (float)NERF_GRIDSIZE - 0.5f) * scale + 0.5f);
	f3 w = div3(sub3(pos, mk3(M.aabb_min[0], M.aabb_min[1], M.aabb_min[2])), mk3(M.aabb_diag[0], M.aabb_diag[1], M.aabb_diag[2]));
	for (int p = 0; p < 4; ++p) {
		const int src = 16 * p + c;
		const float sx = __shfl(w.x, src, 64), sy = __shfl(w.y, src, 64), sz = __shfl(w.z, src, 64);
		const uint32_t s_idx = (uint32_t)__shfl((int)idx, src, 64);
		const int s_valid = __shfl(valid ? 1 : 0, src, 64);
		half8 enc = encode_level_pair(t_grid, t_xgrid, s_lv, lane >> 4, sx, sy, sz);
		half_t logit = density_pass<DLIN>(s_w, lane, enc);
		if (lane < 16 && s_valid) {
			float thickness = network_to_density((float)logit, M.density_act) * stepsize();
			atomicMax((unsigned int*)&grid_tmp[s_idx], __float_as_uint(thickness));
		}
	}
}
__global__ void density_grid_positions_kernel(const ModelParams M, uint32_t n_samples, Pcg32 rng, uint32_t step, uint32_t n_cascades, float thresh,
                                              const float* __restrict__ grid_in, float* __restrict__ pos01, uint32_t* __restrict__ cell) {
	const uint32_t i = blockIdx.x * blockDim.x + threadIdx.x;
	if (i >= n_samples) return;
	rng.advance((uint64_t)i * 4u);
	const uint32_t level = (uint32_t)(rng.next_float() * (float)n_cascades) % n_cascades;
	uint32_t idx = 0;
	for (uint32_t j = 0; j < 10; ++j) {
		idx = ((i + step * n_samples) * 56924617u + j * 19349663u + 96925573u) % NERF_GRID_N_CELLS;
		idx += level * NERF_GRID_N_CELLS;
		if (grid_in[idx] > thresh) break;
	}
	const uint32_t pos_idx = idx % NERF_GRID_N_CELLS;
	const float x = (float)morton3D_invert(pos_idx >> 0), y = (float)morton3D_invert(pos_idx >> 1), z = (float)morton3D_invert(pos_idx >> 2);
	const float rx = rng.next_float(), ry = rng.next_float(), rz = rng.next_float();
	const float scale = __builtin_ldexpf(1.0f, (int)level);
	const f3 pos = mk3(((x + rx) / (float)NERF_GRIDSIZE - 0.5f) * scale + 0.5f, ((y + ry) / (float)NERF_GRIDSIZE - 0.5f) * scale + 0.5f,
	                   ((z + rz) / (float)NERF_GRIDSIZE - 0.5f) * scale + 0.5f);
	const f3 w = div3(sub3(pos, mk3(M.aabb_min[0], M.aabb_min[1], M.aabb_min[2])), mk3(M.aabb_diag[0], M.aabb_diag[1], M.aabb_diag[2]));
	pos01[3 * (size_t)i] = w.x; pos01[3 * (size_t)i + 1] = w.y; pos01[3 * (size_t)i + 2] = w.z;
	cell[i] = idx;
}
__global__ void density_grid_splat_kernel(uint32_t n_samples, uint32_t density_act, const uint32_t* __restrict__ cell, const uint16_t* __restrict__ net_out, float* __restrict__ grid_tmp) {
	const uint32_t i = blockIdx.x * blockDim.x + threadIdx.x;
	if (i >= n_samples) return;
	union { uint16_t u; half_t h; } cv;
	cv.u = net_out[(size_t)i * 4 + 3];
	const float thickness = network_to_density((float)cv.h, density_act) * stepsize();
	atomicMax((unsigned int*)&grid_tmp[cell[i]], __float_as_uint(thickness));
}

__global__ void density_grid_ema_kernel(uint32_t n_elements, float decay, float* __restrict__ grid, const float* __restrict__ grid_tmp) {
	uint32_t i = blockIdx.x * blockDim.x + threadIdx.x;
	if (i >= n_elements) return;
	float prev = grid[i];
	grid[i] = prev < 0.f ? prev : fmaxf(prev * decay, grid_tmp[i]);
}

__global__ void init_rays_kernel(const ModelParams M, const CameraParams C, NerfPayload* __restrict__ payloads) {
	uint32_t x = threadIdx.x + blockDim.x * blockIdx.x;
	uint32_t y = threadIdx.y + blockDim.y * blockIdx.y;
	if (x >= (uint32_t)C.width || y >= (uint32_t)C.height) return;
	RayState r;
	init_ray(M, C, x, y, r);
	advance_pos(M, C, r);
	NerfPayload p;
	p.origin[0] = r.o.x; p.origin[1] = r.o.y; p.origin[2] = r.o.z;
	p.dir[0] = r.d.x; p.dir[1] = r.d.y; p.dir[2] = r.d.z;
	p.t = r.t;
	p.max_weight = 0.f;
	p.idx = r.alive || (r.d.x != 0.f || r.d.y != 0.f || r.d.z != 0.f) ? r.idx : 0u;
	p.n_steps = 0;
	p.alive = r.alive ? 1 : 0;
	p.pad = 0;
	payloads[x + (uint32_t)C.width * y] = p;
}

__global__ void half_to_float_kernel(uint32_t n, const uint16_t* __restrict__ in, float* __restrict__ out) {
	uint32_t i = blockIdx.x * blockDim.x + threadIdx.x;
	if (i >= n) return;
	union { uint16_t u; half_t h; } cv;
	cv.u = in[i];
	out[i] = (float)cv.h;
}

__global__ void density_mean_kernel(uint32_t n, const float* __restrict__ grid, double* __restrict__ partial) {
	__shared__ double s[256];
	double acc = 0.0;
	for (uint32_t i = blockIdx.x * blockDim.x + threadIdx.x; i < n; i += gridDim.x * blockDim.x) acc += (double)(fmaxf(grid[i], 0.0f) / (float)n);
	s[threadIdx.x] = acc;
	__syncthreads();
	for (int off = 128; off > 0; off >>= 1) {
		if ((int)threadIdx.x < off) s[threadIdx.x] += s[threadIdx.x + off];
		__syncthreads();
	}
	if (threadIdx.x == 0) partial[blockIdx.x] = s[0];
}

__global__ void grid_to_bitfield_kernel(uint32_t n_elements, uint32_t n_nonzero_elements, const float* __restrict__ grid, uint8_t* __restrict__ bitfield, float mean) {
	uint32_t i = blockIdx.x * blockDim.x + threadIdx.x;
	if (i >= n_elements) return;
	if (i >= n_nonzero_elements) { bitfield[i] = 0; return; }
	float thresh = fminf(0.01f, mean);
	uint8_t bits = 0;
#pragma unroll
	for (int j = 0; j < 8; ++j) bits |= grid[(size_t)i * 8 + j] > thresh ? (uint8_t)(1u << j) : 0;
	bitfield[i] = bits;
}

__global__ void coarse_occupancy_kernel(const uint8_t* __restrict__ bitfield, uint32_t* __restrict__ coarse) {
	uint32_t w = blockIdx.x * blockDim.x + threadIdx.x;
	if (w >= NERF_CASCADES * COARSE_WORDS_PER_MIP) return;
	const uint2* src = (const uint2*)(bitfield + (size_t)w * 256);
	uint32_t bits = 0;
	for (int b = 0; b < 32; ++b) {
		uint2 v = src[b];
		bits |= ((v.x | v.y) != 0u ? 1u : 0u) << b;
	}
	coarse[w] = bits;
}
__global__ void coarse16_occupancy_kernel(uint32_t* __restrict__ coarse) {
	uint32_t w = threadIdx.x;
	if (w >= NERF_CASCADES * 16) return;
	uint32_t bits = 0;
	for (int b = 0; b < 32; ++b) {
		uint32_t a0 = coarse[(size_t)(w * 32 + b) * 2], a1 = coarse[(size_t)(w * 32 + b) * 2 + 1];
		bits |= ((a0 | a1) != 0u ? 1u : 0u) << b;
	}
	coarse[NERF_CASCADES * COARSE_WORDS_PER_MIP + w] = bits;
}

__global__ void bitfield_max_pool_kernel(uint32_t n_elements, const uint8_t* __restrict__ prev_level, uint8_t* __restrict__ next_level) {
	uint32_t i = blockIdx.x * blockDim.x + threadIdx.x;
	if (i >= n_elements) return;
	uint8_t bits = 0;
#pragma unroll
	for (int j = 0; j < 8; ++j) bits |= prev_level[(size_t)i * 8 + j] > 0 ? (uint8_t)(1u << j) : 0;
	uint32_t x = morton3D_invert(i >> 0) + NERF_GRIDSIZE / 8;
	uint32_t y = morton3D_invert(i >> 1) + NERF_GRIDSIZE / 8;
	uint32_t z = morton3D_invert(i >> 2) + NERF_GRIDSIZE / 8;
	next_level[morton3D(x, y, z)] |= bits;
}

__global__ void accumulate_tonemap_kernel(uint32_t n_pixels, const float4* __restrict__ frame_buffer, float4* __restrict__ accumulate_buffer,
                                          float sample_count, float4 background, float exposure_scale, int to_srgb, int color_space, float4* __restrict__ rgba_out) {
	uint32_t i = blockIdx.x * blockDim.x + threadIdx.x;
	if (i >= n_pixels) return;
	float4 color = frame_buffer[i];
	if (color_space == 1) {
		color.x = linear_to_srgb(color.x);
		color.y = linear_to_srgb(color.y);
		color.z = linear_to_srgb(color.z);
	}
	float4 tmp = sample_count > 0.f ? accumulate_buffer[i] : make_float4(0.f, 0.f, 0.f, 0.f);
	tmp.x = (tmp.x * sample_count + color.x) / (sample_count + 1.0f);
	tmp.y = (tmp.y * sample_count + color.y) / (sample_count + 1.0f);
	tmp.z = (tmp.z * sample_count + color.z) / (sample_count + 1.0f);
	tmp.w = (tmp.w * sample_count + color.w) / (sample_count + 1.0f);
	accumulate_buffer[i] = tmp;
	if (!rgba_out) return;
	float bgr = background.x, bgg = background.y, bgb = background.z;
	if (color_space != 1) {
		bgr = srgb_to_linear(bgr);
		bgg = srgb_to_linear(bgg);
		bgb = srgb_to_linear(bgb);
	}
	float weight = (1.0f - tmp.w) * background.w;
	tmp.x += bgr * weight;
	tmp.y += bgg * weight;
	tmp.z += bgb * weight;
	tmp.w += weight;
	if (color_space == 1) {
		tmp.x = srgb_to_linear(tmp.x);
		tmp.y = srgb_to_linear(tmp.y);
		tmp.z = srgb_to_linear(tmp.z);
	}
	tmp.x *= exposure_scale;
	tmp.y *= exposure_scale;
	tmp.z *= exposure_scale;
	if (to_srgb) {
		tmp.x = linear_to_srgb(tmp.x);
		tmp.y = linear_to_srgb(tmp.y);
		tmp.z = linear_to_srgb(tmp.z);
	}
	rgba_out[i] = tmp;
}

template <typename K>
static int resident_blocks_per_cu(K kernel) {
	int n = 0;
	if (hipOccupancyMaxActiveBlocksPerMultiprocessor(&n, kernel, BLOCK, 0) != hipSuccess || n < 1) n = 1;
	return n;
}
static int grid_blocks(const FrameParams& F, int resident) {
	const int waves = BLOCK / 64, needed = (int)((F.n_local_tiles + waves - 1) / waves);
	return resident > needed ? (needed > 0 ? needed : 1) : resident;
}
static FrameParams with_grid(const FrameParams& F, int n_blocks) {
	FrameParams G = F;
	G.n_waves = (uint32_t)n_blocks * (BLOCK / 64);
	return G;
}
static int head_kind(const ModelParams& M) { return M.rgb_mid < 0 ? (M.density_linear ? -2 : -1) : M.rgb_mid; }

enum RenderKernel { RK_GENERIC, RK_UNIT, RK_UNIT_PLAIN, RK_C5, RK_C5_PLAIN, RK_PROF, RK_UNIT_PLAIN_PROF, RK_UNIT_PLAIN_PROF2,
                    RK_MID0, RK_MID2, RK_LIN_RGB, RK_LIN, RK_NORMALS, RK_COUNT, RK_WIDE = RK_COUNT };
static RenderKernel select_render_kernel(const ModelParams& M, const CameraParams& C, const FrameParams& F) {
	if (M.wide.width) return RK_WIDE;
	if (F.render_mode == 7) return RK_NORMALS;
	switch (head_kind(M)) {
	case -2: return RK_LIN;
	case -1: return RK_LIN_RGB;
	case 0: return RK_MID0;
	case 2: return RK_MID2;
	}
	const bool unit = M.max_cascade == 0 && M.cone_angle <= 1e-5f;
	const bool c5 = !unit && M.max_cascade < 5 && !F.outside_possible;
	const bool plain = C.lens_mode == 0 && C.aperture_size == 0.0f && !C.moving && !F.envmap;
	bool stamped = F.prof != nullptr;
#ifdef NGP_EXPERIMENT_CELL_CACHE_STATS
	stamped = stamped && F.prof_level > 0;
#endif
	if (stamped) return unit && plain ? (F.prof_level >= 2 ? RK_UNIT_PLAIN_PROF2 : RK_UNIT_PLAIN_PROF) : RK_PROF;
	if (unit) return plain ? RK_UNIT_PLAIN : RK_UNIT;
	if (c5) return plain ? RK_C5_PLAIN : RK_C5;
	return RK_GENERIC;
}
static const struct { void (*kernel)(ModelParams, CameraParams, FrameParams); bool clamped; } RENDER_KERNELS[RK_COUNT] = {
	{render_nerf_fused, true}, {render_nerf_fused_unit, true}, {render_nerf_fused_unit_plain, true}, {render_nerf_fused_c5, true},
	{render_nerf_fused_c5_plain, true}, {render_nerf_fused_prof, true}, {render_nerf_fused_unit_plain_prof, true},
	{render_nerf_fused_unit_plain_prof2, true}, {render_nerf_fused_mid0, false}, {render_nerf_fused_mid2, false},
	{render_nerf_fused_lin_rgb, false}, {render_nerf_fused_lin, false}, {render_nerf_fused_normals, false}};
static const char* const RENDER_KERNEL_NAMES[RK_COUNT + 1] = {
	"render_nerf_fused", "render_nerf_fused_unit", "render_nerf_fused_unit_plain", "render_nerf_fused_c5", "render_nerf_fused_c5_plain", "render_nerf_fused_prof",
	"render_nerf_fused_unit_plain_prof", "render_nerf_fused_unit_plain_prof2", "render_nerf_fused_mid0", "render_nerf_fused_mid2", "render_nerf_fused_lin_rgb",
	"render_nerf_fused_lin", "render_nerf_fused_normals", "wide"};
void launch_render_nerf_wide(const ModelParams& M, const CameraParams& C, const FrameParams& F, int n_cus, hipStream_t stream);
void launch_trace_probe_wide(const ModelParams& M, const FrameParams& F, const ProbeParams& P, int n_cus, hipStream_t stream);
const char* launch_render_nerf(const ModelParams& M, const CameraParams& C, const FrameParams& F, int n_cus, hipStream_t stream) {
	const RenderKernel k = select_render_kernel(M, C, F);
	if (k == RK_WIDE) {
		launch_render_nerf_wide(M, C, F, n_cus, stream);
		return RENDER_KERNEL_NAMES[k];
	}
	static const struct PerCu { int v[RK_COUNT]; } resident = []() {
		PerCu r;
		for (int i = 0; i < RK_COUNT; ++i) r.v[i] = resident_blocks_per_cu(RENDER_KERNELS[i].kernel);
		return r;
	}();
	int per_cu = resident.v[k];
	if (RENDER_KERNELS[k].clamped) {
		static const int shard_per_cu = []() { const char* e = getenv("NGP_SHARD_BLOCKS_PER_CU"); int v = e ? atoi(e) : 2; return v >= 1 && v <= 8 ? v : 2; }();
		if (F.shard_count > 1 && per_cu > shard_per_cu) per_cu = shard_per_cu;
		if (F.shard_count <= 1 && F.n_local_tiles <= 6144u && per_cu > 2) per_cu = 2;
		if (const char* e = getenv("NGP_BLOCKS_PER_CU")) { int v = atoi(e); if (v > 0 && v < per_cu) per_cu = v; }
	}
	const int n_blocks = grid_blocks(F, n_cus * per_cu);
	const FrameParams G = with_grid(F, n_blocks);
	hipLaunchKernelGGL(RENDER_KERNELS[k].kernel, dim3(n_blocks), dim3(BLOCK), 0, stream, M, C, G);
	return RENDER_KERNEL_NAMES[k];
}
void launch_trace_probe(const ModelParams& M, const FrameParams& F, const ProbeParams& P, int n_cus, hipStream_t stream) {
	if (M.wide.width) return launch_trace_probe_wide(M, F, P, n_cus, stream);
	static const int per_cu = resident_blocks_per_cu(trace_probe_fused);
	const int n_blocks = grid_blocks(F, n_cus * per_cu);
	const FrameParams G = with_grid(F, n_blocks);
	hipLaunchKernelGGL(trace_probe_fused, dim3(n_blocks), dim3(BLOCK), 0, stream, M, G, P);
}
void launch_probe_reduce(const ProbeParams& P, float4* envmap, hipStream_t stream) {
	uint32_t n = P.n_theta * P.n_phi * (P.mode == 3 ? P.grid_x * P.grid_y : 1u);
	hipLaunchKernelGGL(probe_reduce_kernel, dim3((n + 127) / 128), dim3(128), 0, stream, P, envmap);
}
void launch_irradiance(const ProbeParams& P, const float4* envmap, uint32_t n, const float* normals, float4* out, hipStream_t stream) {
	IrradianceQuery Q{};
	Q.n_theta = P.n_theta; Q.n_phi = P.n_phi;
	Q.envmap = envmap;
	Q.n = n;
	Q.normals = normals;
	Q.outward = P.mode == 1 ? 1 : (P.mode == 3 ? 3 : 0);
	for (int i = 0; i < 3; ++i) { Q.origin[i] = P.origin[i]; Q.center[i] = P.center[i]; }
	Q.grid_x = P.grid_x; Q.grid_y = P.grid_y; Q.shell_radius = P.shell_radius;
	Q.out = out;
	if (n) hipLaunchKernelGGL(irradiance_kernel, dim3(n), dim3(256), 0, stream, Q);
// ... 92 lines not shown
```

surface-irradiance-estimation-from-neural-radiance-fields_amd/csrc/ngp_kernels.h:

```cpp
#pragma once

#include <hip/hip_runtime.h>
#include <stdint.h>

namespace ngp {

constexpr uint32_t NERF_GRIDSIZE = 128;
constexpr uint32_t NERF_GRID_N_CELLS = NERF_GRIDSIZE * NERF_GRIDSIZE * NERF_GRIDSIZE;
constexpr uint32_t NERF_CASCADES = 8;
constexpr uint32_t NERF_STEPS = 1024;
constexpr float MAX_DEPTH = 16384.0f;
constexpr uint32_t MARCH_ITER = 10000;

constexpr int N_LEVELS = 8;
constexpr int N_FEATURES = 4;
constexpr int MLP_WIDTH = 64;
constexpr int FRAG_D0 = 0, FRAG_D1 = 4, FRAG_R0 = 6, FRAG_R1 = 10, FRAG_R2 = 18, N_FRAGS = 20;
constexpr int MAX_RGB_MID = 2, N_FRAGS_MAX = FRAG_R1 + 8 * MAX_RGB_MID + 2;
constexpr int n_frags_for(int rgb_mid) { return rgb_mid < 0 ? FRAG_R0 + 1 : FRAG_R1 + 8 * rgb_mid + 2; }
constexpr int N_NORMALS_FRAGS = 4, FRAG_NORMALS = N_FRAGS_MAX;

struct LevelInfo {
	float scale;
	uint32_t res;
	uint32_t size;
	uint32_t offset;
	uint32_t hashed;
	uint32_t mask;
	uint32_t coord_max;
	uint32_t mul_y8, mul_z8, mask8, base8;
	uint32_t xor_disabled;
};
static_assert(sizeof(LevelInfo) == 48, "LevelInfo layout");

struct NerfPayload {
	float origin[3];
	float dir[3];
	float t;
	float max_weight;
	uint32_t idx;
	uint16_t n_steps;
	uint8_t alive;
	uint8_t pad;
};
static_assert(sizeof(NerfPayload) == 40, "NerfPayload layout");

constexpr int WIDE_TILE_M = 32;
constexpr int WIDE_TILE_K = 16;
constexpr int WIDE_MAX_LAYERS = 24;
struct WideLayer {
	uint32_t frag_offset;
	uint16_t n_kblocks;
	uint16_t n_mtiles;
};
struct WideModel {
	const uint4* frags;
	uint32_t width;
	uint32_t pos_freqs, dir_freqs;
	uint32_t pos_identity, dir_identity;
	uint32_t enc_dims, dir_dims, rgb_in;
	uint32_t n_hidden_density, n_hidden_rgb;
	WideLayer layers[WIDE_MAX_LAYERS];
	WideLayer layers_t[8];
	uint32_t out_row0_offset;
};
constexpr int WIDE_MAX_NORMALS_LAYERS = 8;

struct ModelParams {
	const uint2* grid;
	const char* xgrid;
	const uint4* wfrags;
	const uint8_t* bitfield;
	const uint32_t* coarse;
	LevelInfo levels[N_LEVELS];
	float aabb_min[3], aabb_diag[3];
	float raabb_min[3], raabb_max[3];
	float r2l[9];
	uint32_t max_cascade;
	float cone_angle;
	uint32_t rgb_act, density_act;
	int32_t rgb_mid;
	uint32_t density_linear;
	uint32_t r2l_identity;
	uint32_t diag_pow2;
	float aabb_inv_diag[3];
	uint32_t grid_bytes, xgrid_bytes;
	WideModel wide;
};
constexpr uint32_t COARSE_WORDS_PER_MIP = 32 * 32 * 32 / 32;

struct CameraParams {
	float m[12];
	int32_t width, height;
	float focal[2];
	float screen_center[2];
	float pixel_offset[2];
	uint32_t spp;
	float near_distance;
	int32_t lens_mode;
	float lens_params[7];
	float aperture_size, focus_z;
	float m1[12];
	float rolling_shutter[4];
	int32_t moving;
};

struct FrameParams {
	float4* frame_buffer;
	float* depth_buffer;
	uint32_t* queue;
	uint32_t* xqueue;
	unsigned long long* counters;
	unsigned long long* results;
	uint32_t* done;
	uint32_t n_waves;
	int32_t add_results;
	uint32_t tiles_x, tiles_y;
	uint32_t n_local_tiles;
	uint32_t shard_index, shard_count;
	float min_transmittance;
	int32_t linear_colors;
	int32_t depth_test;
	int32_t packed;
	int32_t tune[8];
	int32_t outside_possible;
	int32_t render_mode;
	float depth_scale;
	int32_t direct, to_srgb, color_space;
	float background[4];
	float exposure_scale;
	const float4* envmap;
	int32_t env_w, env_h;
	unsigned long long* prof;
	uint32_t* trace;
	uint32_t trace_stride, trace_cap_waves, trace_cap_iters;
	int32_t prof_level;
};

struct ProbeParams {
	int32_t mode;
	uint32_t n_theta, n_phi, n_origin;
	float origin[3];
	float center[3];
	uint32_t n_rays;
	float4* ray_rgba;
	uint32_t grid_x, grid_y;
	float shell_radius;
	const float* ray_o;
	const float* ray_d;
	const float2* ray_t;
	float* ray_depth;
};
constexpr int32_t PROBE_RAY_LIST = 4;

struct Triangle {
	float a[3], b[3], c[3];
};
struct TriangleBvhNode {
	float bmin[3], bmax[3];
	int left_idx;
	int right_idx;
};
struct MeshRef {
	const TriangleBvhNode* nodes;
	const Triangle* tris;
	float bmin[3], bmax[3];
	uint32_t n_tris, n_nodes;
};
struct MeshSceneParams {
	const MeshRef* meshes;
	uint32_t n_meshes;
	float scene_min[3], scene_max[3];
};
struct MeshShadeParams {
	float sun_dir[3], up_dir[3];
	float metallic, subsurface, specular, roughness, sheen, clearcoat, clearcoat_gloss;
	float basecolor[3], ambientcolor[3];
};
struct IrradianceMap {
	const float4* irradiance;
	uint32_t n_theta, n_phi;
	uint32_t grid_x, grid_y;
	float center[3];
};

}
```

surface-irradiance-estimation-from-neural-radiance-fields_amd/csrc/ngp_model.cpp:

```cpp
#include "ngp_host.h"

#include <algorithm>
#include <cmath>
#include <cstring>

using namespace ngp;

namespace {

uint32_t next_multiple(uint32_t v, uint32_t d) { return ((v + d - 1) / d) * d; }

void build_levels(const ngp_model_desc& d, LevelInfo* lv, uint32_t* total_entries) {
	float log2_pls = log2f(d.per_level_scale);
	uint32_t offset = 0;
	for (uint32_t l = 0; l < d.n_levels; ++l) {
		float scale = exp2f((float)l * log2_pls) * (float)d.base_resolution - 1.0f;
		if (!(scale >= 0.0f && scale < 1073741824.0f)) throw std::runtime_error("invalid hash grid configuration (a level's resolution is out of range)");
		uint32_t res = (uint32_t)ceilf(scale) + 1u;
		uint32_t max_params = 0xFFFFFFFFu / 2u;
		uint32_t n = powf((float)res, 3.0f) > (float)max_params ? max_params : res * res * res;
		n = next_multiple(n, 8u);
		n = std::min(n, 1u << d.log2_hashmap_size);
		uint32_t stride = 1;
		for (int dim = 0; dim < 3 && stride <= n; ++dim) stride *= res;
// ... 115 lines not shown
	return L;
}

struct WideShapes {
	uint32_t alignment, enc_dims, dir_dims, rgb_in, rgb_out;
};
WideShapes wide_shapes(const ngp_model_desc& d) {
	WideShapes w{};
	w.alignment = d.mlp_alignment ? d.mlp_alignment : 16u;
	auto up = [&](uint32_t v) { return (v + w.alignment - 1) / w.alignment * w.alignment; };
	w.enc_dims = d.pos_encoding == 2 ? up(3u) : up(6u * d.pos_n_frequencies);
	w.dir_dims = d.dir_encoding == 1 ? up(6u * d.dir_n_frequencies) : d.dir_encoding == 2 ? up(3u) : 16u;
	w.rgb_in = up(d.density_out_dims + w.dir_dims);
	w.rgb_out = up(3u);
	return w;
}

struct ModelLayout {
	uint64_t nd, nr, ng;
	uint32_t max_cascade;
	WideShapes ws;
	LevelInfo levels[N_LEVELS];
};

ModelLayout validate_model_desc(const ngp_model_desc& d) {
	const bool wide = d.pos_encoding >= 1;
	if (d.pos_encoding > 2 || d.dir_encoding > 2 || (d.mlp_alignment != 0 && d.mlp_alignment != 8 && d.mlp_alignment != 16)) throw std::runtime_error("invalid model descriptor (encoding kinds / mlp_alignment)");
	if (!wide && d.dir_encoding != 0) throw std::runtime_error("unsupported network architecture: a Frequency / Identity direction encoding is implemented together with a Frequency / Identity position encoding (configs/nerf/frequency.json, none.json)");
	if (wide) {
		if ((d.n_neurons != 128 && d.n_neurons != 256) || d.n_hidden_density < 1 || d.n_hidden_rgb < 1 || d.n_hidden_density + d.n_hidden_rgb + 2 > (uint32_t)WIDE_MAX_LAYERS ||
		    d.density_out_dims != 16 || (d.pos_encoding == 1 && (d.pos_n_frequencies < 1 || d.pos_n_frequencies > 40)) || (d.dir_encoding == 1 && (d.dir_n_frequencies < 1 || d.dir_n_frequencies > 4))) {
			throw std::runtime_error("unsupported network architecture: with a Frequency position encoding (configs/nerf/frequency.json) the HIP path implements MLPs of 128 or 256 "
			                         "neurons with 1 or more hidden layers, a 16-wide density output, up to 40 position and 4 direction frequencies");
		}
	} else if (d.n_levels != N_LEVELS || d.n_features_per_level != N_FEATURES || d.n_neurons != MLP_WIDTH || d.n_hidden_density > 1 ||
	           d.n_hidden_rgb > 1 + (uint32_t)MAX_RGB_MID || d.density_out_dims != 16 || (d.n_hidden_density == 0 && d.n_hidden_rgb != 0)) {
		throw std::runtime_error("unsupported network architecture: the HIP path is specialised for configs/nerf/base.json and its variants "
		                         "(HashGrid 8 levels x 4 features; density MLP 64x1 hidden -> 16 with an rgb MLP 64 wide of 0 to 3 hidden layers -- "
		                         "base, base_0layer .. base_3layer --, or both heads without a hidden layer -- linear.json)");
	}
	if (!wide && ((d.log2_hashmap_size > 28 && d.log2_hashmap_size != 31) || d.base_resolution == 0 || !(d.per_level_scale > 0.f))) throw std::runtime_error("invalid hash grid configuration");
	if (d.aabb_scale == 0 || (d.aabb_scale & (d.aabb_scale - 1)) != 0) throw std::runtime_error("NeRF dataset's `aabb_scale` must be a power of two");
	if (d.aabb_scale > (1u << (NERF_CASCADES - 1))) throw std::runtime_error("NeRF dataset must have `aabb_scale <= 128`");

	ModelLayout L{};
	uint32_t total_entries = 0;
	if (!wide) build_levels(d, L.levels, &total_entries);
	L.ws = wide_shapes(d);
	const uint32_t enc_dims = wide ? L.ws.enc_dims : d.n_levels * d.n_features_per_level;
	L.nd = mlp_n_params(enc_dims, d.n_neurons, d.n_hidden_density, d.density_out_dims);
	L.nr = wide ? mlp_n_params(L.ws.rgb_in, d.n_neurons, d.n_hidden_rgb, L.ws.rgb_out) : mlp_n_params(d.density_out_dims + 16u, d.n_neurons, d.n_hidden_rgb, L.ws.rgb_out);
	L.ng = wide ? 0 : (uint64_t)total_entries * d.n_features_per_level;
	if (d.n_params != L.nd + L.nr + L.ng || !d.params_fp16) {
		throw std::runtime_error("parameter count mismatch: snapshot has " + std::to_string(d.n_params) + ", network needs " + std::to_string(L.nd + L.nr + L.ng));
	}
	while ((1u << L.max_cascade) < d.aabb_scale) ++L.max_cascade;
	if (d.n_density_grid != 0 && d.n_density_grid != (uint64_t)NERF_GRID_N_CELLS * (L.max_cascade + 1)) throw std::runtime_error("Incompatible number of grid cascades.");
	return L;
}

void upload_wide_weights(ngp_ctx* ctx, const ngp_model_desc& d, const WideShapes& ws, WideModel& WM) {
	std::vector<uint16_t> frags;
	WM.width = d.n_neurons;
	WM.pos_freqs = d.pos_encoding == 1 ? d.pos_n_frequencies : 0u;
	WM.dir_freqs = d.dir_encoding == 1 ? d.dir_n_frequencies : 0u;
	WM.pos_identity = d.pos_encoding == 2 ? 1u : 0u;
	WM.dir_identity = d.dir_encoding == 2 ? 1u : 0u;
	WM.enc_dims = ws.enc_dims;
	WM.dir_dims = ws.dir_dims;
	WM.rgb_in = ws.rgb_in;
	WM.n_hidden_density = d.n_hidden_density;
	WM.n_hidden_rgb = d.n_hidden_rgb;
	const uint16_t* W = ctx->params.data();
	uint32_t l = 0;
	auto emit_mlp = [&](uint32_t n_in, uint32_t n_hidden, uint32_t n_out) {
		WM.layers[l++] = emit_wide_fragments(frags, W, d.n_neurons, n_in);
		W += (size_t)d.n_neurons * n_in;
		for (uint32_t k = 1; k < n_hidden; ++k) {
			WM.layers[l++] = emit_wide_fragments(frags, W, d.n_neurons, d.n_neurons);
			W += (size_t)d.n_neurons * d.n_neurons;
		}
		WM.layers[l++] = emit_wide_fragments(frags, W, n_out, d.n_neurons);
		W += (size_t)n_out * d.n_neurons;
	};
	emit_mlp(ws.enc_dims, d.n_hidden_density, d.density_out_dims);
	emit_mlp(ws.rgb_in, d.n_hidden_rgb, ws.rgb_out);
	if (d.n_hidden_density <= (uint32_t)WIDE_MAX_NORMALS_LAYERS) {
		const uint16_t* D = ctx->params.data();
		std::vector<uint16_t> wt((size_t)d.n_neurons * d.n_neurons);
		uint32_t n_in = ws.enc_dims;
		for (uint32_t k = 0; k < d.n_hidden_density; ++k) {
			std::fill(wt.begin(), wt.end(), (uint16_t)0);
			for (uint32_t o = 0; o < d.n_neurons; ++o)
				for (uint32_t i = 0; i < n_in && i < d.n_neurons; ++i) wt[(size_t)i * d.n_neurons + o] = D[(size_t)o * n_in + i];
			WM.layers_t[k] = emit_wide_fragments(frags, wt.data(), d.n_neurons, d.n_neurons);
			D += (size_t)d.n_neurons * n_in;
			n_in = d.n_neurons;
		}
		WM.out_row0_offset = (uint32_t)(frags.size() / 8);
		frags.insert(frags.end(), D, D + d.n_neurons);
	}
	ctx->d_wfrags.upload((const uint4*)frags.data(), frags.size() / 8);
	WM.frags = ctx->d_wfrags.get();
}

void upload_grid_tables(ngp_ctx* ctx, const ngp_model_desc& d, const ModelLayout& L, ModelParams& M) {
	const uint64_t nd = L.nd, nr = L.nr, ng = L.ng;
	memcpy(M.levels, L.levels, sizeof(M.levels));
	ctx->d_params.upload(ctx->params.data() + nd + nr, ng);
	{
		std::vector<uint64_t> table;
		build_xor_layout(M.levels, d.n_levels, ctx->params.data() + nd + nr, table);
		ctx->d_xgrid.upload(table.data(), table.size());
		if (table.size() * sizeof(uint64_t) > 0x7FFFFFFFull || ng * sizeof(uint16_t) > 0x7FFFFFFFull) throw std::runtime_error("hash grid too large for 31-bit buffer-load offsets");
		M.xgrid_bytes = (uint32_t)(table.size() * sizeof(uint64_t));
		M.grid_bytes = (uint32_t)(ng * sizeof(uint16_t));
	}
	std::vector<uint16_t> frags((size_t)(N_FRAGS_MAX + N_NORMALS_FRAGS) * 64 * 8, 0);
	const uint16_t* W = ctx->params.data();
	if (d.n_hidden_density == 0) {
		emit_fragments(frags, FRAG_D0, W, 16, 32);
	} else {
		emit_fragments(frags, FRAG_D0, W, 64, 32);
		emit_fragments(frags, FRAG_D1, W + 64 * 32, 16, 64);
	}
	const uint16_t* R = W + nd;
	const int rgb_mid = (int)d.n_hidden_rgb - 1;
	if (rgb_mid < 0) {
		emit_fragments(frags, FRAG_R0, R, (int)L.ws.rgb_out, 32);
	} else {
		emit_fragments(frags, FRAG_R0, R, 64, 32);
		for (int k = 0; k < rgb_mid; ++k) emit_fragments(frags, FRAG_R1 + 8 * k, R + 64 * 32 + (size_t)k * 64 * 64, 64, 64);
		emit_fragments(frags, FRAG_R1 + 8 * rgb_mid, R + 64 * 32 + (size_t)rgb_mid * 64 * 64, (int)L.ws.rgb_out, 64);
	}
	M.rgb_mid = rgb_mid;
	M.density_linear = d.n_hidden_density == 0 ? 1u : 0u;
	ctx->d_wfrags.upload((const uint4*)frags.data(), frags.size() / 8);
	launch_build_normals_fragments(ctx->d_wfrags.get(), ctx->stream);
}

void upload_occupancy(ngp_ctx* ctx, const ngp_model_desc& d, uint32_t max_cascade) {
	const uint64_t n_grid_expected = (uint64_t)NERF_GRID_N_CELLS * (max_cascade + 1);
	const size_t bitfield_bytes = (size_t)NERF_GRID_N_CELLS / 8 * NERF_CASCADES;
	ctx->d_bitfield.reset(bitfield_bytes);
	ctx->d_density_f32.reset(n_grid_expected);
	ctx->d_partial.reset(256);
	if (d.n_density_grid) {
		ctx->d_density_f16.upload(ctx->density_grid.data(), d.n_density_grid);
	} else {
		NGP_HIP_CHECK(hipMemset(ctx->d_density_f32.get(), 0, n_grid_expected * sizeof(float)));
	}
	launch_density_grid_to_bitfield(ctx->d_density_f16.get(), (uint32_t)d.n_density_grid, max_cascade, ctx->d_density_f32.get(), ctx->d_partial.get(), ctx->d_bitfield.get(),
	                                &ctx->bitfield_mean, ctx->stream);
	ctx->d_coarse.reset((size_t)NERF_CASCADES * COARSE_WORDS_PER_MIP + NERF_CASCADES * 16);
	launch_coarse_occupancy(ctx->d_bitfield.get(), ctx->d_coarse.get(), ctx->stream);
	NGP_HIP_CHECK(hipStreamSynchronize(ctx->stream));
	NGP_HIP_CHECK(hipGetLastError());
}

void fill_model_params(const ngp_ctx* ctx, const ngp_model_desc& d, uint32_t max_cascade, ModelParams& M) {
	M.grid = (const uint2*)ctx->d_params.get();
	M.xgrid = (const char*)ctx->d_xgrid.get();
	M.coarse = ctx->d_coarse.get();
	M.wfrags = d.pos_encoding >= 1 ? nullptr : ctx->d_wfrags.get();
	M.bitfield = ctx->d_bitfield.get();
	for (int i = 0; i < 3; ++i) {
		M.aabb_min[i] = d.aabb_min[i];
		M.aabb_diag[i] = d.aabb_max[i] - d.aabb_min[i];
		M.raabb_min[i] = d.render_aabb_min[i];
		M.raabb_max[i] = d.render_aabb_max[i];
	}
	for (int i = 0; i < 9; ++i) M.r2l[i] = d.render_aabb_to_local[i];
	{
		const float ident[9] = {1, 0, 0, 0, 1, 0, 0, 0, 1};
		M.r2l_identity = memcmp(M.r2l, ident, sizeof(ident)) == 0 ? 1u : 0u;
		M.diag_pow2 = 1u;
		for (int i = 0; i < 3; ++i) {
			int e;
			float m = frexpf(M.aabb_diag[i], &e);
			if (!(m == 0.5f) || e < -100 || e > 100) M.diag_pow2 = 0u;
			M.aabb_inv_diag[i] = 1.0f / M.aabb_diag[i];
		}
	}
	M.max_cascade = max_cascade;
	M.cone_angle = d.cone_angle_constant;
	M.rgb_act = d.rgb_activation;
	M.density_act = d.density_activation;
}

}

namespace ngp {
void free_model(ngp_ctx* ctx) {
	free_training(ctx);
	ctx->d_params.reset();
	ctx->d_xgrid.reset();
	ctx->d_wfrags.reset();
	ctx->d_bitfield.reset();
	ctx->d_coarse.reset();
	ctx->d_density_f16.reset();
	ctx->d_density_f32.reset();
	ctx->d_density_tmp.reset();
	ctx->d_partial.reset();
	ctx->model_loaded = false;
}

void set_model_impl(ngp_ctx* ctx, const ngp_model_desc& d) {
	const ModelLayout L = validate_model_desc(d);

	if (ctx->device >= 0) NGP_HIP_CHECK(hipDeviceSynchronize());
	free_model(ctx);
	ctx->params.assign(d.params_fp16, d.params_fp16 + d.n_params);
	ctx->density_grid.assign(d.density_grid_fp16, d.density_grid_fp16 + d.n_density_grid);
	ctx->desc = d;
	ctx->desc.params_fp16 = nullptr;
	ctx->desc.density_grid_fp16 = nullptr;
	ctx->max_cascade = L.max_cascade;
	ctx->have_desc = true;
	{
		Pcg32 rng;
		rng.seed(1337u);
		Pcg32 grid_rng;
		grid_rng.seed(rng.next_uint());
		ctx->grid_rng_state = grid_rng.state;
		ctx->grid_rng_inc = grid_rng.inc;
		ctx->grid_ema_step = 0;
		ctx->grid_updates = 0;
	}
	if (ctx->device < 0) return;

	ModelParams M{};
	if (d.pos_encoding >= 1) upload_wide_weights(ctx, d, L.ws, M.wide);
	else upload_grid_tables(ctx, d, L, M);
	upload_occupancy(ctx, d, L.max_cascade);
	fill_model_params(ctx, d, L.max_cascade, M);
	ctx->M = M;
	ctx->model_loaded = true;
	++ctx->model_generation;
	ctx->grid_generation = ctx->params_generation = 0;
}

void update_density_grid_device(ngp_ctx* ctx, float decay, uint32_t n_uniform, uint32_t n_nonuniform, uint32_t n_iterations) {
	const uint32_t n_cascades = ctx->max_cascade + 1;
	const uint32_t n_elements = NERF_GRID_N_CELLS * n_cascades;
	hipStream_t stream = ctx->stream;
	ensure_frame_buffers(ctx, 0);
	order_after_frames(ctx, stream);
	if (!ctx->d_density_tmp) ctx->d_density_tmp.reset(n_elements);
	Pcg32 rng;
	rng.state = ctx->grid_rng_state;
	rng.inc = ctx->grid_rng_inc;
	for (uint32_t it = 0; it < n_iterations; ++it) {
		uint32_t nu = n_uniform, nn = n_nonuniform;
		if (nu == 0 && nn == 0) {
			if (ctx->grid_updates < 256) nu = NERF_GRID_N_CELLS * n_cascades;
			else nu = nn = NERF_GRID_N_CELLS / 4 * n_cascades;
		}
		NGP_HIP_CHECK(hipMemsetAsync(ctx->d_density_tmp.get(), 0, (size_t)n_elements * sizeof(float), stream));
		if (ctx->M.wide.width) {
			const size_t n_max = std::max(nu, nn);
			if (n_max * 24 > ctx->d_grid_scratch.size()) ctx->d_grid_scratch.reset(n_max * 24);
			float* d_pos = (float*)ctx->d_grid_scratch.get();
			uint32_t* d_cell = (uint32_t*)(ctx->d_grid_scratch.get() + n_max * 12);
			uint16_t* d_out = (uint16_t*)(ctx->d_grid_scratch.get() + n_max * 16);
			launch_density_grid_update_wide(ctx->M, nu, rng, ctx->grid_ema_step, n_cascades, -0.01f, ctx->d_density_f32.get(), ctx->d_density_tmp.get(), d_pos, d_cell, d_out, ctx->n_cus, stream);
			rng.advance();
			launch_density_grid_update_wide(ctx->M, nn, rng, ctx->grid_ema_step, n_cascades, 0.01f, ctx->d_density_f32.get(), ctx->d_density_tmp.get(), d_pos, d_cell, d_out, ctx->n_cus, stream);
			rng.advance();
		} else {
			launch_density_grid_update(ctx->M, nu, rng, ctx->grid_ema_step, n_cascades, -0.01f, ctx->d_density_f32.get(), ctx->d_density_tmp.get(), stream);
			rng.advance();
			launch_density_grid_update(ctx->M, nn, rng, ctx->grid_ema_step, n_cascades, 0.01f , ctx->d_density_f32.get(), ctx->d_density_tmp.get(), stream);
			rng.advance();
		}
		launch_density_grid_ema(n_elements, decay, ctx->d_density_f32.get(), ctx->d_density_tmp.get(), stream);
		++ctx->grid_ema_step;
		++ctx->grid_updates;
	}
	ctx->grid_rng_state = rng.state;
	ctx->grid_rng_inc = rng.inc;
	launch_density_grid_to_bitfield(nullptr, 0, ctx->max_cascade, ctx->d_density_f32.get(), ctx->d_partial.get(), ctx->d_bitfield.get(), &ctx->bitfield_mean, stream);
	launch_coarse_occupancy(ctx->d_bitfield.get(), ctx->d_coarse.get(), stream);
	mark_model_updated(ctx, stream);
	ctx->density_grid_host_dirty = true;
	++ctx->grid_generation;
}
void refresh_density_grid_host(ngp_ctx* ctx) {
	if (!ctx->density_grid_host_dirty || ctx->device < 0 || !ctx->model_loaded) return;
	const uint32_t n_elements = NERF_GRID_N_CELLS * (ctx->max_cascade + 1);
	std::vector<float> grid(n_elements);
	NGP_HIP_CHECK(hipMemcpyAsync(grid.data(), ctx->d_density_f32.get(), (size_t)n_elements * sizeof(float), hipMemcpyDeviceToHost, ctx->stream));
	NGP_HIP_CHECK(hipStreamSynchronize(ctx->stream));
	NGP_HIP_CHECK(hipGetLastError());
	ctx->density_grid.resize(n_elements);
	for (uint32_t i = 0; i < n_elements; ++i) ctx->density_grid[i] = float_to_half(grid[i]);
	ctx->desc.n_density_grid = n_elements;
	ctx->density_grid_host_dirty = false;
}
}

extern "C" {

int ngp_set_model(ngp_ctx* ctx, const ngp_model_desc* desc) {
	return guarded(ctx, [&] {
		if (!desc) throw std::runtime_error("null model descriptor");
		set_model_impl(ctx, *desc);
		ctx->config = mj::Value();
// ... 67 lines not shown
```

surface-irradiance-estimation-from-neural-radiance-fields_amd/csrc/ngp_multi.cpp:

```cpp
#include "ngp_host.h"

#include <cstring>

namespace ngp {

void launch_unpack_tiles(const float4* gathered_rgba, const float* gathered_depth, uint32_t n_devices, uint32_t n_slots, int width, int height, float4* rgba, float* depth,
                         hipStream_t stream);

namespace {
void sync_peer_model(ngp_ctx* primary, ngp_ctx* peer) {
	sync_inference_model(primary);
	if (peer->synced_generation != primary->model_generation || !peer->model_loaded) {
		sync_host_params(primary);
		refresh_density_grid_host(primary);
		ngp_model_desc d = primary->desc;
		d.params_fp16 = primary->params.data();
		d.n_params = primary->params.size();
		d.density_grid_fp16 = primary->density_grid.data();
		d.n_density_grid = primary->density_grid.size();
		{
			DeviceGuard g(peer->device);
			set_model_impl(peer, d);
		}
		peer->synced_generation = primary->model_generation;
		peer->synced_grid_generation = primary->grid_generation == 0 ? 0 : ~0ull;
		peer->synced_params_generation = primary->params_generation == 0 ? 0 : ~0ull;
	}
	const bool grid = peer->synced_grid_generation != primary->grid_generation, params = peer->synced_params_generation != primary->params_generation;
	if (!grid && !params) return;
	{
		DeviceGuard g(primary->device);
		if (!primary->ev_model_valid) mark_model_updated(primary, primary->stream);
	}
	DeviceGuard g(peer->device);
	hipStream_t s = peer->stream;
	NGP_HIP_CHECK(hipStreamWaitEvent(s, primary->ev_model, 0));
	order_after_frames(peer, s);
	if (grid) {
		const size_t n_cells = (size_t)NERF_GRID_N_CELLS * (primary->max_cascade + 1);
		NGP_HIP_CHECK(hipMemcpyPeerAsync(peer->d_bitfield.get(), peer->device, primary->d_bitfield.get(), primary->device, (size_t)NERF_GRID_N_CELLS / 8 * NERF_CASCADES, s));
		NGP_HIP_CHECK(hipMemcpyPeerAsync(peer->d_coarse.get(), peer->device, primary->d_coarse.get(), primary->device, ((size_t)NERF_CASCADES * COARSE_WORDS_PER_MIP + NERF_CASCADES * 16) * sizeof(uint32_t), s));
		NGP_HIP_CHECK(hipMemcpyPeerAsync(peer->d_density_f32.get(), peer->device, primary->d_density_f32.get(), primary->device, n_cells * sizeof(float), s));
		peer->bitfield_mean = primary->bitfield_mean;
		peer->grid_rng_state = primary->grid_rng_state;
		peer->grid_rng_inc = primary->grid_rng_inc;
		peer->grid_ema_step = primary->grid_ema_step;
		peer->grid_updates = primary->grid_updates;
		peer->synced_grid_generation = primary->grid_generation;
	}
	if (params) {
		NGP_HIP_CHECK(hipMemcpyPeerAsync(peer->d_params.get(), peer->device, primary->d_params.get(), primary->device, primary->M.grid_bytes, s));
		NGP_HIP_CHECK(hipMemcpyPeerAsync(peer->d_xgrid.get(), peer->device, primary->d_xgrid.get(), primary->device, primary->M.xgrid_bytes, s));
		NGP_HIP_CHECK(hipMemcpyPeerAsync(peer->d_wfrags.get(), peer->device, primary->d_wfrags.get(), primary->device, (size_t)(N_FRAGS_MAX + N_NORMALS_FRAGS) * 64 * sizeof(uint4), s));
		peer->synced_params_generation = primary->params_generation;
	}
	mark_model_updated(peer, s);
	if (!peer->ev_synced) peer->ev_synced = new_event(hipEventDisableTiming);
	NGP_HIP_CHECK(hipEventRecord(peer->ev_synced, s));
	{
		DeviceGuard gp(primary->device);
		NGP_HIP_CHECK(hipStreamWaitEvent(primary->stream, peer->ev_synced, 0));
	}
}

void ensure_pair(DevArray<float4>& rgba, DevArray<float>& depth, size_t n) {
	if (n <= depth.size()) return;
	rgba.reset(), depth.reset();
	rgba.reset(n);
	depth.reset(n);
}

void enable_peer_access(int dev, int peer) {
	try {
		DeviceGuard g(dev);
		(void)hipDeviceEnablePeerAccess(peer, 0);
	} catch (const std::exception&) {
	}
	(void)hipGetLastError();
}

void ensure_pack_buffers(ngp_ctx* ctx, size_t n_pixels_packed) {
	ensure_pair(ctx->d_pack_rgba, ctx->d_pack_depth, n_pixels_packed);
	if (!ctx->ev_pack) ctx->ev_pack = new_event(hipEventDisableTiming);
}
}

void render_frames_multi(ngp_ctx* ctx, const ngp_camera& cam, const ngp_render_opts& opts, float4* d_rgba, float* d_depth, hipStream_t stream) {
	if (opts.packed_output) throw std::runtime_error("packed_output addresses one shard: render it through a single-device context");
	const uint32_t n_dev = 1u + (uint32_t)ctx->peers.size();
	const uint32_t n_slots = tile_share(cam.width, cam.height, 0, n_dev);
	const size_t packed = (size_t)n_slots * 64;
	{
		DeviceGuard g(ctx->device);
		ensure_pair(ctx->d_gather_rgba, ctx->d_gather_depth, packed * n_dev);
		if (!ctx->ev_pack) ctx->ev_pack = new_event(hipEventDisableTiming);
		if (ctx->n_multi_frames > 0) NGP_HIP_CHECK(hipStreamWaitEvent(stream, ctx->ev_unpacked, 0));
		NGP_HIP_CHECK(hipEventRecord(ctx->ev_pack, stream));
	}
	for (uint32_t i = 0; i < n_dev; ++i) {
		ngp_ctx* dev = i == 0 ? ctx : ctx->peers[i - 1];
		if (i > 0) {
			if (ctx->model_loaded) sync_peer_model(ctx, dev);
			memcpy(dev->M.raabb_min, ctx->M.raabb_min, sizeof(ctx->M.raabb_min));
			memcpy(dev->M.raabb_max, ctx->M.raabb_max, sizeof(ctx->M.raabb_max));
			memcpy(dev->M.r2l, ctx->M.r2l, sizeof(ctx->M.r2l));
			dev->M.r2l_identity = ctx->M.r2l_identity;
			dev->M.cone_angle = ctx->M.cone_angle;
			memcpy(dev->tune, ctx->tune, sizeof(ctx->tune));
			if (opts.testbed_mode == NGP_MODE_GEOMETRY) sync_peer_geometry(ctx, dev);
		}
		DeviceGuard g(dev->device);
		ensure_pack_buffers(dev, packed);
		hipStream_t s = i == 0 ? stream : dev->stream;
		ngp_render_opts o = opts;
		o.shard_index = i;
		o.shard_count = n_dev;
		o.packed_output = 1;
		if (i > 0) NGP_HIP_CHECK(hipStreamWaitEvent(s, ctx->ev_pack, 0));
		render_frames(dev, cam, o, dev->d_pack_rgba.get(), dev->d_pack_depth.get(), s);
		NGP_HIP_CHECK(hipMemcpyPeerAsync(ctx->d_gather_rgba.get() + packed * i, ctx->device, dev->d_pack_rgba.get(), dev->device, packed * sizeof(float4), s));
		NGP_HIP_CHECK(hipMemcpyPeerAsync(ctx->d_gather_depth.get() + packed * i, ctx->device, dev->d_pack_depth.get(), dev->device, packed * sizeof(float), s));
		if (i > 0) NGP_HIP_CHECK(hipEventRecord(dev->ev_pack, s));
	}
	DeviceGuard g(ctx->device);
	for (ngp_ctx* p : ctx->peers) NGP_HIP_CHECK(hipStreamWaitEvent(stream, p->ev_pack, 0));
	if (!d_depth) {
		ensure_frame_buffers(ctx, (size_t)cam.width * cam.height);
		d_depth = ctx->d_depth.get();
	}
	launch_unpack_tiles(ctx->d_gather_rgba.get(), ctx->d_gather_depth.get(), n_dev, n_slots, cam.width, cam.height, d_rgba, d_depth, stream);
	if (!ctx->ev_unpacked) ctx->ev_unpacked = new_event(hipEventDisableTiming);
	NGP_HIP_CHECK(hipEventRecord(ctx->ev_unpacked, stream));
	++ctx->n_multi_frames;
	ctx->last_was_multi = true;
	NGP_HIP_CHECK(hipGetLastError());
}

}

extern "C" {

ngp_ctx* ngp_create_multi(const int* devices, int n_devices) {
	if (!devices || n_devices < 1 || n_devices > 64) return nullptr;
	ngp_ctx* primary = ngp_create(devices[0]);
	if (!primary) return nullptr;
	for (int i = 1; i < n_devices; ++i) {
		ngp_ctx* p = ngp_create(devices[i]);
		if (!p) {
			ngp_destroy(primary);
			return nullptr;
		}
		p->primary = primary;
		primary->peers.push_back(p);
		if (devices[i] != devices[0]) {
			int can = 0;
			(void)hipDeviceCanAccessPeer(&can, devices[0], devices[i]);
			if (can) {
				ngp::enable_peer_access(devices[0], devices[i]);
				ngp::enable_peer_access(devices[i], devices[0]);
			}
		}
	}
	(void)hipSetDevice(devices[0]);
	return primary;
}

int ngp_n_devices(const ngp_ctx* ctx) { return ctx ? 1 + (int)ctx->peers.size() : 0; }

int ngp_get_device_render_stats(ngp_ctx* ctx, int device_index, ngp_render_stats* out) {
	return ngp::guarded(ctx, [&] {
		if (!out || device_index < 0 || device_index > (int)ctx->peers.size()) throw std::runtime_error("invalid argument");
		ngp_ctx* dev = device_index == 0 ? ctx : ctx->peers[device_index - 1];
		ngp::DeviceGuard g(dev->device);
		const bool multi = dev->last_was_multi;
		dev->last_was_multi = false;
		const int rc = ngp_get_render_stats(dev, out);
		dev->last_was_multi = multi;
		if (rc != 0) throw std::runtime_error(dev->error);
	});
}

}
```

surface-irradiance-estimation-from-neural-radiance-fields_amd/csrc/wide_kernels.hip:

```cpp
#include "render_common.h"

#include <cstdio>
#include <cstdlib>

namespace ngp {

constexpr int WBLOCK = 256;
constexpr int ROWS = 128;
constexpr int XS = 264;
constexpr int DIR_STRIDE = 24;
typedef float floatx16 __attribute__((ext_vector_type(16)));

struct WideShared {
	half_t x[ROWS * XS];
	half_t dir[WBLOCK * DIR_STRIDE];
	uint16_t owner[ROWS];
	uint32_t cnt[8];
	uint32_t coarse16[NERF_CASCADES * 16];
	unsigned long long prof[16];
};
NGP_DEV float4* row_meta(WideShared& S, int row) { return (float4*)(S.x + row * XS + 256); }
static_assert(2 * sizeof(WideShared) <= 160 * 1024, "two workgroups per CU");

NGP_DEV uint32_t empty_block_size_global(f3 pos, const uint8_t* __restrict__ bitfield, const uint32_t* s_coarse16, uint32_t mip, OccBlockCache& cache) {
	float mip_scale = __builtin_ldexpf(1.0f, -(int)mip);
	pos = adds3(scale3(adds3(pos, -0.5f), mip_scale), 0.5f);
	int ix = (int)(pos.x * (float)NERF_GRIDSIZE);
	int iy = (int)(pos.y * (float)NERF_GRIDSIZE);
	int iz = (int)(pos.z * (float)NERF_GRIDSIZE);
	if (ix < 0 || ix >= (int)NERF_GRIDSIZE || iy < 0 || iy >= (int)NERF_GRIDSIZE || iz < 0 || iz >= (int)NERF_GRIDSIZE) return 1u;
	const uint32_t idx = morton3D((uint32_t)ix, (uint32_t)iy, (uint32_t)iz);
	const uint32_t b16 = idx >> 12;
	if (!((s_coarse16[mip * 16u + (b16 >> 5)] >> (b16 & 31u)) & 1u)) return 16u;
	const uint32_t b4 = idx >> 6, key = (mip << 26) | b4;
	if (cache.key != key) {
		cache.bits = *(const uint2*)(bitfield + (size_t)b4 * 8 + (size_t)(NERF_GRID_N_CELLS / 8) * mip);
		cache.key = key;
	}
	if ((cache.bits.x | cache.bits.y) == 0u) return 4u;
	const uint32_t word = (idx & 32u) ? cache.bits.y : cache.bits.x;
	return ((word >> (idx & 31u)) & 1u) ? 0u : 1u;
}

NGP_DEV floatx16 mfma32(half8 a, half8 b, floatx16 c) { return __builtin_amdgcn_mfma_f32_32x32x16_f16(a, b, c, 0, 0, 0); }

NGP_DEV float encoder_sin_reduced(float t) {
	const float k = __builtin_rintf(t * 0.318309886183790672f);
	float r = __builtin_fmaf(-k, 3.14159274101257324f, t);
	r = __builtin_fmaf(-k, -8.74227765734758577e-08f, r);
	r = __builtin_fmaf(-k, -3.55271367880050093e-15f, r);
	const float r2 = r * r;
	float p = -2.50521083854417188e-08f;
	p = __builtin_fmaf(p, r2, 2.75573192239858907e-06f);
	p = __builtin_fmaf(p, r2, -1.98412698412698413e-04f);
	p = __builtin_fmaf(p, r2, 8.33333333333333333e-03f);
	p = __builtin_fmaf(p, r2, -1.66666666666666667e-01f);
	const float s = __builtin_fmaf(r * r2, p, r);
	const uint32_t flip = (uint32_t)(int)k << 31;
	return __builtin_bit_cast(float, __builtin_bit_cast(uint32_t, s) ^ flip);
}
NGP_DEV float encoder_sin(float t) {
	if (!(__builtin_fabsf(t) < 1048576.0f)) return sinf(t);
	return encoder_sin_reduced(t);
}
NGP_DEV float encoder_cos(float t) {
	if (!(__builtin_fabsf(t) < 1048576.0f)) return cosf(t);
	const float k = __builtin_rintf(t * 0.318309886183790672f);
	float r = __builtin_fmaf(-k, 3.14159274101257324f, t);
	r = __builtin_fmaf(-k, -8.74227765734758577e-08f, r);
	r = __builtin_fmaf(-k, -3.55271367880050093e-15f, r);
	const float r2 = r * r;
	float p = 2.08767569878680990e-09f;
	p = __builtin_fmaf(p, r2, -2.75573192239858907e-07f);
	p = __builtin_fmaf(p, r2, 2.48015873015873016e-05f);
	p = __builtin_fmaf(p, r2, -1.38888888888888889e-03f);
	p = __builtin_fmaf(p, r2, 4.16666666666666667e-02f);
	p = __builtin_fmaf(p, r2, -0.5f);
	const float c = __builtin_fmaf(p, r2, 1.0f);
	const uint32_t flip = (uint32_t)(int)k << 31;
	return __builtin_bit_cast(float, __builtin_bit_cast(uint32_t, c) ^ flip);
}

NGP_DEV void frequency_encode(uint32_t n_freq, uint32_t padded, float x, float y, float z, half_t* out, uint32_t f_begin, uint32_t f_end, bool tail, uint32_t k_end = 0) {
	const float PI = 3.14159265358979323846f;
	const float in[3] = {x, y, z};
	if (n_freq <= 16u && __builtin_fabsf(x) <= 8.0f && __builtin_fabsf(y) <= 8.0f && __builtin_fabsf(z) <= 8.0f) {
		for (uint32_t f = f_begin; f < f_end; ++f) {
#pragma unroll
			for (int d = 0; d < 3; ++d) {
				const float v = __builtin_ldexpf(in[d], (int)f);
				half2_t sc;
				sc[0] = (half_t)encoder_sin_reduced(__builtin_fmaf(v, PI, 0.0f));
				sc[1] = (half_t)encoder_sin_reduced(__builtin_fmaf(v, PI, PI / 2.0f));
				*(half2_t*)(out + (uint32_t)d * 2u * n_freq + 2u * f) = sc;
			}
		}
	} else {
#pragma unroll
		for (int d = 0; d < 3; ++d) {
			for (uint32_t f = f_begin; f < f_end; ++f) {
				const float v = __builtin_ldexpf(in[d], (int)f);
				half2_t sc;
				sc[0] = (half_t)encoder_sin(__builtin_fmaf(v, PI, 0.0f));
				sc[1] = (half_t)encoder_sin(__builtin_fmaf(v, PI, PI / 2.0f));
				*(half2_t*)(out + (uint32_t)d * 2u * n_freq + 2u * f) = sc;
			}
		}
	}
	if (tail) {
		const half2_t ones = {(half_t)1.0f, (half_t)1.0f};
		for (uint32_t j = 6u * n_freq; j < padded; j += 2u) *(half2_t*)(out + j) = ones;
		const half8 zeros = {0, 0, 0, 0, 0, 0, 0, 0};
		for (uint32_t j = padded; j < k_end; j += 8u) *(half8*)(out + j) = zeros;
	}
}

NGP_DEV void identity_encode(uint32_t padded, float x, float y, float z, half_t* out, uint32_t k_end = 0) {
	half8 v = {(half_t)x, (half_t)y, (half_t)z, (half_t)1.0f, (half_t)1.0f, (half_t)1.0f, (half_t)1.0f, (half_t)1.0f};
	*(half8*)out = v;
	const half8 ones = {(half_t)1.0f, (half_t)1.0f, (half_t)1.0f, (half_t)1.0f, (half_t)1.0f, (half_t)1.0f, (half_t)1.0f, (half_t)1.0f};
	for (uint32_t j = 8u; j < padded; j += 8u) *(half8*)(out + j) = ones;
	const half8 zeros = {0, 0, 0, 0, 0, 0, 0, 0};
	for (uint32_t j = padded; j < k_end; j += 8u) *(half8*)(out + j) = zeros;
}

NGP_DEV uint2 pack4(float a, float b, float c, float d, bool relu) {
	half2_t lo = {(half_t)a, (half_t)b}, hi = {(half_t)c, (half_t)d};
	if (relu) {
		const half2_t zero = {(half_t)0.0f, (half_t)0.0f};
		lo = __builtin_elementwise_max(lo, zero);
		hi = __builtin_elementwise_max(hi, zero);
	}
	return make_uint2(__builtin_bit_cast(uint32_t, lo), __builtin_bit_cast(uint32_t, hi));
}

typedef unsigned int u32x4 __attribute__((ext_vector_type(4)));
constexpr int RING = 3, AHEAD = RING - 1;
NGP_DEV void lds_barrier() { asm volatile("s_waitcnt lgkmcnt(0)\n\ts_barrier" ::: "memory"); }
NGP_DEV half8 as_half8(u32x4 u) { return __builtin_bit_cast(half8, u); }

struct LayerFrags {
	const uint4* base;
	int nkb, mt;
};
template <int MT>
NGP_DEV void ring_preload(u32x4 (&ar)[RING][MT], LayerFrags L) {
#pragma unroll
	for (int st = 0; st < AHEAD; ++st)
#pragma unroll
		for (int m = 0; m < MT; ++m)
			if (m < L.mt) ar[st][m] = *(const u32x4*)(L.base + ((size_t)m * L.nkb + st) * 64);
}

template <int MT, int NKB, int MODE = 0>
NGP_DEV void wide_hidden_layer(half_t* X, u32x4 (&ar)[RING][MT], const uint4* __restrict__ wf, int wave, int lane, LayerFrags next, unsigned long long* pr = nullptr, uint8_t* mask = nullptr) {
	const int n = lane & 31, h = lane >> 5;
	unsigned long long ts0 = 0;
	if (pr) ts0 = stamp();
	const floatx16 zero = {0.f, 0.f, 0.f, 0.f, 0.f, 0.f, 0.f, 0.f, 0.f, 0.f, 0.f, 0.f, 0.f, 0.f, 0.f, 0.f};
	floatx16 acc[MT][4];
	const half_t* col = X + n * XS + 8 * h;
	half8 b[2][4];
#pragma unroll
	for (int t = 0; t < 4; ++t) b[0][t] = *(const half8*)(col + 32 * t * XS);
#pragma unroll
	for (int kb = 0; kb < NKB; ++kb) {
		if (kb + AHEAD < NKB) {
#pragma unroll
			for (int m = 0; m < MT; ++m) ar[(kb + AHEAD) % RING][m] = *(const u32x4*)(wf + ((size_t)m * NKB + kb + AHEAD) * 64);
		}
		if (kb + 1 < NKB) {
#pragma unroll
			for (int t = 0; t < 4; ++t) b[(kb + 1) & 1][t] = *(const half8*)(col + 32 * t * XS + 16 * (kb + 1));
		}
		__builtin_amdgcn_sched_barrier(0);
		if (kb == NKB - 1) lds_barrier();
#pragma unroll
		for (int t = 0; t < 4; ++t)
#pragma unroll
			for (int m = 0; m < MT; ++m) acc[m][t] = mfma32(as_half8(ar[kb % RING][m]), b[kb & 1][t], kb == 0 ? zero : acc[m][t]);
		if (kb < NKB - 1) __builtin_amdgcn_sched_barrier(0);
	}
	ring_preload<MT>(ar, next);
#pragma unroll
	for (int t = 0; t < 4; ++t) {
		half_t* row = X + (32 * t + n) * XS + 32 * (wave * MT) + 8 * h;
// ... 697 lines not shown
```

Baseline: 1116 Mrays/s.

## Index occupancy summaries linearly and defer opaque-ray normalization to retire

Replaces Morton indexing of the 4^3 and 16^3 occupancy summary tables with linear x|y|z bit packing. It also adds a linearly indexed copy of the 64-bit per-block occupancy words after the summary tables, so the march lookup reuses its cache key directly and skips a Morton encode. The per-ray division that normalizes an opaque ray's colour is moved out of the composite loop into the retire/shade step, tracked with a wave ballot mask. The old behaviour is kept behind an NGP_ROUND_V1 build variant, and the extra table enlarges the coarse buffer.

```diff
diff --git a/__graft_entry__.py b/__graft_entry__.py
--- a/__graft_entry__.py
+++ b/__graft_entry__.py
@@ -17,6 +17,7 @@
     _pkg("build").build(legacy=True)
     _pkg("build").build(nocache=True)
     _pkg("build").build(netsec_v1=True)
+    _pkg("build").build(round_v1=True)
     _pkg("build").build_pyngp()
     _pkg("build").build_main()
     sys.path.insert(0, os.path.join(ROOT, "oracle"))
diff --git a/surface-irradiance-estimation-from-neural-radiance-fields_amd/build.py b/surface-irradiance-estimation-from-neural-radiance-fields_amd/build.py
--- a/surface-irradiance-estimation-from-neural-radiance-fields_amd/build.py
+++ b/surface-irradiance-estimation-from-neural-radiance-fields_amd/build.py
@@ -19,6 +19,7 @@
 LIB_LEGACY = os.path.join(HERE, "libngp_hip_legacy.so")
 LIB_CELLSTATS = os.path.join(HERE, "libngp_hip_cellstats.so")
 LIB_NOCACHE = os.path.join(HERE, "libngp_hip_nocache.so")
+LIB_ROUND_V1 = os.path.join(HERE, "libngp_hip_round_v1.so")
 LIB_NETSEC_V1 = os.path.join(HERE, "libngp_hip_netsec_v1.so")
 
 
@@ -33,15 +34,15 @@
     return os.path.getmtime(inc) > t
 
 
-def build(force=False, verbose=False, legacy=False, nocache=False, cellstats=False, netsec_v1=False):
-    if legacy + nocache + cellstats + netsec_v1 > 1:
+def build(force=False, verbose=False, legacy=False, nocache=False, cellstats=False, netsec_v1=False, round_v1=False):
+    if legacy + nocache + cellstats + netsec_v1 + round_v1 > 1:
         raise ValueError("one variant at a time")
-    lib = LIB_LEGACY if legacy else LIB_NOCACHE if nocache else LIB_CELLSTATS if cellstats else LIB_NETSEC_V1 if netsec_v1 else LIB
+    lib = LIB_LEGACY if legacy else LIB_NOCACHE if nocache else LIB_CELLSTATS if cellstats else LIB_NETSEC_V1 if netsec_v1 else LIB_ROUND_V1 if round_v1 else LIB
     if not force and not needs_build(lib):
         return lib
     srcs = [os.path.join(CSRC, s) for s in SOURCES if os.path.exists(os.path.join(CSRC, s))]
     tmp = "%s.%d.tmp" % (lib, os.getpid())
-    cmd = [hipcc()] + FLAGS + (["-DNGP_TCNN_LEGACY_ENCODE"] if legacy else []) + (["-DNGP_NO_CELL_CACHE"] if nocache else []) + (["-DNGP_EXPERIMENT_CELL_CACHE_STATS"] if cellstats else []) + (["-DNGP_NETSEC_V1"] if netsec_v1 else []) + os.environ.get("NGP_BUILD_DEFINES", "").split() + ["-o", tmp] + srcs + ["-lz"]
+    cmd = [hipcc()] + FLAGS + (["-DNGP_TCNN_LEGACY_ENCODE"] if legacy else []) + (["-DNGP_NO_CELL_CACHE"] if nocache else []) + (["-DNGP_EXPERIMENT_CELL_CACHE_STATS"] if cellstats else []) + (["-DNGP_NETSEC_V1"] if netsec_v1 else []) + (["-DNGP_ROUND_V1"] if round_v1 else []) + os.environ.get("NGP_BUILD_DEFINES", "").split() + ["-o", tmp] + srcs + ["-lz"]
     if verbose:
         print(" ".join(cmd))
     r = subprocess.run(cmd, capture_output=True, text=True)
diff --git a/surface-irradiance-estimation-from-neural-radiance-fields_amd/csrc/nerf_device.h b/surface-irradiance-estimation-from-neural-radiance-fields_amd/csrc/nerf_device.h
--- a/surface-irradiance-estimation-from-neural-radiance-fields_amd/csrc/nerf_device.h
+++ b/surface-irradiance-estimation-from-neural-radiance-fields_amd/csrc/nerf_device.h
@@ -2,6 +2,7 @@
 
 #include "ngp_kernels.h"
 #include "cell_cache.h"
+#include "occ_index.h"
 
 namespace ngp {
 
@@ -124,6 +125,16 @@
 	return dt * (max_stepsize - stepsize()) + stepsize();
 }
 
+typedef unsigned int u32x2 __attribute__((ext_vector_type(2)));
+typedef __amdgpu_buffer_rsrc_t GridRsrc;
+NGP_DEV GridRsrc make_grid_rsrc(const void* table, uint32_t bytes) { return __builtin_amdgcn_make_buffer_rsrc(const_cast<void*>(table), (short)0, (int)bytes, 0x00020000); }
+NGP_DEV uint2 gather8(GridRsrc r, uint32_t offset) {
+	const u32x2 v = __builtin_amdgcn_raw_buffer_load_b64(r, (int)offset, 0, 0);
+	return make_uint2(v.x, v.y);
+}
+static_assert(OCC_GRIDSIZE == NERF_GRIDSIZE && OCC_SUMMARY4_WORDS_PER_MIP == COARSE_WORDS_PER_MIP && COARSE_SUMMARY_WORDS % 2 == 0, "occ_index.h and ngp_kernels.h describe the same tables");
+NGP_DEV const uint2* occ_words(const uint32_t* __restrict__ coarse) { return (const uint2*)(coarse + COARSE_SUMMARY_WORDS); }
+
 NGP_DEV uint32_t expand_bits(uint32_t v) {
 	v = (v * 0x00010001u) & 0xFF0000FFu;
 	v = (v * 0x00000101u) & 0x0F00F00Fu;
@@ -160,8 +171,8 @@
 	int iz = (int)(pos.z * (float)NERF_GRIDSIZE);
 	if (ix < 0 || ix >= (int)NERF_GRIDSIZE || iy < 0 || iy >= (int)NERF_GRIDSIZE || iz < 0 || iz >= (int)NERF_GRIDSIZE) return false;
 	uint32_t idx = morton3D((uint32_t)ix, (uint32_t)iy, (uint32_t)iz);
-	uint32_t block = idx >> 6;
-	if (!((s_coarse[mip * COARSE_WORDS_PER_MIP + (block >> 5)] >> (block & 31u)) & 1u)) return false;
+	uint32_t block = occ_block4((uint32_t)ix, (uint32_t)iy, (uint32_t)iz);
+	if (!((s_coarse[occ_summary4_word(mip, block)] >> (block & 31u)) & 1u)) return false;
 	return (bitfield[idx / 8 + (NERF_GRID_N_CELLS / 8) * mip] & (1u << (idx % 8))) != 0;
 }
 
@@ -179,10 +190,10 @@
 	int iz = (int)(pos.z * (float)NERF_GRIDSIZE);
 	if (ix < 0 || ix >= (int)NERF_GRIDSIZE || iy < 0 || iy >= (int)NERF_GRIDSIZE || iz < 0 || iz >= (int)NERF_GRIDSIZE) return 1u;
 	uint32_t idx = morton3D((uint32_t)ix, (uint32_t)iy, (uint32_t)iz);
-	uint32_t b16 = idx >> 12;
-	if (!((s_coarse16[mip * 16u + (b16 >> 5)] >> (b16 & 31u)) & 1u)) return 16u;
-	uint32_t b4 = idx >> 6;
-	if (!((s_coarse[mip * COARSE_WORDS_PER_MIP + (b4 >> 5)] >> (b4 & 31u)) & 1u)) return 4u;
+	uint32_t b16 = occ_block16((uint32_t)ix, (uint32_t)iy, (uint32_t)iz);
+	if (!((s_coarse16[occ_summary16_word(mip, b16)] >> (b16 & 31u)) & 1u)) return 16u;
+	uint32_t b4 = idx >> 6, s4 = occ_block4((uint32_t)ix, (uint32_t)iy, (uint32_t)iz);
+	if (!((s_coarse[occ_summary4_word(mip, s4)] >> (s4 & 31u)) & 1u)) return 4u;
 	const uint32_t key = (mip << 26) | b4;
 	if (cache.key != key) {
 		cache.bits = *(const uint2*)(bitfield + (size_t)b4 * 8 + (size_t)(NERF_GRID_N_CELLS / 8) * mip);
@@ -207,14 +218,22 @@
 	const uint32_t x = (uint32_t)ix, y = (uint32_t)iy, z = (uint32_t)iz;
 	const uint32_t key = (x >> 2) | ((y >> 2) << 5) | ((z >> 2) << 10) | (mip << 15);
 	if (cache.key != key) {
+#ifdef NGP_ROUND_V1
 		const uint32_t b4 = morton3D(x >> 2, y >> 2, z >> 2), b16 = b4 >> 6;
-		if (!((s_coarse16[mip * 16u + (b16 >> 5)] >> (b16 & 31u)) & 1u)) return 16u;
-		const uint32_t cw = mip < lds_mips ? s_coarse[mip * COARSE_WORDS_PER_MIP + (b4 >> 5)] : g_coarse[mip * COARSE_WORDS_PER_MIP + (b4 >> 5)];
+#else
+		const uint32_t b4 = key & (OCC_BLOCKS_PER_MIP - 1u), b16 = occ_block16(x, y, z);
+#endif
+		if (!((s_coarse16[occ_summary16_word(mip, b16)] >> (b16 & 31u)) & 1u)) return 16u;
+		const uint32_t cw = mip < lds_mips ? s_coarse[occ_summary4_word(mip, b4)] : g_coarse[occ_summary4_word(mip, b4)];
 		if (!((cw >> (b4 & 31u)) & 1u)) return 4u;
+#ifdef NGP_ROUND_V1
 		cache.bits = *(const uint2*)(bitfield + (size_t)b4 * 8 + (size_t)(NERF_GRID_N_CELLS / 8) * mip);
+#else
+		cache.bits = occ_words(g_coarse)[occ_block_word(mip, b4)];
+#endif
 		cache.key = key;
 	}
-	const uint32_t bit = (x & 1u) | ((y & 1u) << 1) | ((z & 1u) << 2) | ((x & 2u) << 2) | ((y & 2u) << 3) | ((z & 2u) << 4);
+	const uint32_t bit = occ_bit_in_block(x, y, z);
 	const uint32_t word = (bit & 32u) ? cache.bits.y : cache.bits.x;
 	return ((word >> (bit & 31u)) & 1u) ? 0u : 1u;
 }
@@ -225,9 +244,9 @@
 	pos = adds3(scale3(adds3(pos, -0.5f), mip_scale), 0.5f);
 	const int ix = (int)(pos.x * (float)(NERF_GRIDSIZE / 4)), iy = (int)(pos.y * (float)(NERF_GRIDSIZE / 4)), iz = (int)(pos.z * (float)(NERF_GRIDSIZE / 4));
 	if (((uint32_t)ix | (uint32_t)iy | (uint32_t)iz) >= NERF_GRIDSIZE / 4 || pos.x < 0.0f || pos.y < 0.0f || pos.z < 0.0f) return 0u;
-	const uint32_t b4 = morton3D((uint32_t)ix, (uint32_t)iy, (uint32_t)iz), b16 = b4 >> 6;
-	if (!((s_coarse16[mip * 16u + (b16 >> 5)] >> (b16 & 31u)) & 1u)) return 16u;
-	const uint32_t cw = mip < lds_mips ? s_coarse[mip * COARSE_WORDS_PER_MIP + (b4 >> 5)] : g_coarse[mip * COARSE_WORDS_PER_MIP + (b4 >> 5)];
+	const uint32_t b4 = occ_block4_of_block((uint32_t)ix, (uint32_t)iy, (uint32_t)iz), b16 = occ_block16_of_block((uint32_t)ix, (uint32_t)iy, (uint32_t)iz);
+	if (!((s_coarse16[occ_summary16_word(mip, b16)] >> (b16 & 31u)) & 1u)) return 16u;
+	const uint32_t cw = mip < lds_mips ? s_coarse[occ_summary4_word(mip, b4)] : g_coarse[occ_summary4_word(mip, b4)];
 	return ((cw >> (b4 & 31u)) & 1u) ? 0u : 4u;
 }
 
@@ -641,13 +660,6 @@
 	}
 }
 
-typedef unsigned int u32x2 __attribute__((ext_vector_type(2)));
-typedef __amdgpu_buffer_rsrc_t GridRsrc;
-NGP_DEV GridRsrc make_grid_rsrc(const void* table, uint32_t bytes) { return __builtin_amdgcn_make_buffer_rsrc(const_cast<void*>(table), (short)0, (int)bytes, 0x00020000); }
-NGP_DEV uint2 gather8(GridRsrc r, uint32_t offset) {
-	const u32x2 v = __builtin_amdgcn_raw_buffer_load_b64(r, (int)offset, 0, 0);
-	return make_uint2(v.x, v.y);
-}
 
 typedef _Float16 half2_t __attribute__((ext_vector_type(2)));
 NGP_DEV half_t to_half_rn(float v) {
diff --git a/surface-irradiance-estimation-from-neural-radiance-fields_amd/csrc/nerf_kernels.hip b/surface-irradiance-estimation-from-neural-radiance-fields_amd/csrc/nerf_kernels.hip
--- a/surface-irradiance-estimation-from-neural-radiance-fields_amd/csrc/nerf_kernels.hip
+++ b/surface-irradiance-estimation-from-neural-radiance-fields_amd/csrc/nerf_kernels.hip
@@ -103,6 +103,7 @@
 	occ_cache.key = 0xffffffffu;
 	occ_cache.bits = make_uint2(0u, 0u);
 	bool finished = false;
+	unsigned long long norm_mask = 0ull;
 	bool idle = false;
 	const uint32_t my_wave = threadIdx.x >> 6;
 
@@ -137,17 +138,23 @@
 	};
 	for (;;) {
 		if (PROF) { t0 = stamp(); tr_t[0] = t0; tr_info0 = tr_info1 = tr_march = 0; for (int k = 0; k < 7; ++k) tr_net[k] = 0; }
+		NGP_SECTION("retire");
 		unsigned long long dead_mask = __ballot(!ray.alive);
 		int n_dead = __popcll(dead_mask);
 		if ((exhausted || n_dead >= F.tune[0]) && __any(finished)) {
 			bool hit = false;
 			if (finished) {
+#ifndef NGP_ROUND_V1
+				if ((norm_mask >> lane) & 1ull) { acc.r /= acc.a; acc.g /= acc.a; acc.b /= acc.a; acc.a /= acc.a; }
+#endif
 				hit = shade_ray<PROBE, PLAIN, NORMALS>(F, P, bg_linear, ray.out, acc, step - 1u, ray.d);
 				finished = false;
 			}
+			norm_mask = 0ull;
 			n_hit += (uint32_t)__popcll(__ballot(hit));
 			if (PROF) tr_info1 |= 4u << 24;
 		}
+		NGP_SECTION("refill");
 		if (!exhausted && n_dead >= (F.tune[0] > 16 ? F.tune[0] : 16)) {
 			const uint32_t want = (uint32_t)n_dead >> 4, n_strips = F.n_local_tiles * 4u;
 			uint32_t first = 0, limit = n_strips;
@@ -252,6 +259,7 @@
 			}
 		}
 
+		NGP_SECTION("share");
 		if (!PROBE && F.tune[7] && n_slots == 0u) {
 			const uint32_t st = __hip_atomic_load(&s_xstate, __ATOMIC_RELAXED, __HIP_MEMORY_SCOPE_WORKGROUP);
 			const unsigned long long live_mask = __ballot(ray.alive);
@@ -285,6 +293,7 @@
 				}
 			}
 		}
+		NGP_SECTION("other");
 		if (PROF) { t1 = stamp(); pt[0] += t1 - t0; t0 = t1; tr_t[1] = t1; }
 		const int n_live = __popcll(__ballot(ray.alive));
 		const int k_fit = n_live <= 8 ? 8 : (n_live <= 10 ? 6 : (n_live <= 12 ? 5 : (n_live <= 16 ? 4 : (n_live <= 21 ? 3 : 2))));
@@ -302,6 +311,7 @@
 			if (PROBE && ray.t >= t_max) out = true;
 			const bool inside = marching && !out;
 			uint32_t mip = 0, empty = 1u;
+			NGP_SECTION("march.lookup");
 			if (inside) {
 				if (!UNIT) {
 					mip = mip_from_pos(pos, NERF_CASCADES - 1);
@@ -309,6 +319,7 @@
 				}
 				empty = occupancy_state_at(pos, M.bitfield, s_coarse, s_coarse16, mip, occ_cache, MIPS, M.coarse);
 			}
+			NGP_SECTION("march.emit");
 			const bool emit = inside && empty == 0u;
 			const bool skip = inside && empty != 0u;
 			float e_dt = 0.f;
@@ -320,6 +331,7 @@
 				else e_w = div3(e_w, adiag);
 			}
 			bool ends = marching && out;
+			NGP_SECTION("march.skip");
 			if (skip) {
 				if (!UNIT) {
 					if (PROBE || !F.tune[6]) {
@@ -354,6 +366,7 @@
 				}
 				++skip_i;
 			}
+			NGP_SECTION("march");
 			if (ends) {
 				if (n_pend == 0) {
 					ray.alive = false;
@@ -362,6 +375,7 @@
 					left_box = true;
 				}
 			}
+			NGP_SECTION("march.compact");
 			const unsigned long long emit_mask = __ballot(emit);
 			if (emit_mask) {
 				const uint32_t slot = n_slots + lanes_below(emit_mask);
@@ -589,6 +603,7 @@
 			NGP_SECTION("composite");
 			const bool have = k < n_pend && ray.alive;
 			if (!__any(have)) break;
+			bool ended_opaque = false;
 			if (have) {
 				const uint32_t slot = ((k < 4u ? sl_lo >> (8u * k) : sl_hi >> (8u * (k - 4u))) & 0xffu);
 				const float4 a = s_samp[wave_base + slot];
@@ -631,13 +646,20 @@
 				}
 				++step;
 				if (acc.a > (1.0f - F.min_transmittance)) {
+					NGP_SECTION("composite.end");
+#ifdef NGP_ROUND_V1
 					acc.r /= acc.a; acc.g /= acc.a; acc.b /= acc.a; acc.a /= acc.a;
+#else
+					ended_opaque = true;
+#endif
 					ray.alive = false;
 					finished = true;
+					NGP_SECTION("composite");
 				} else if (step >= MARCH_ITER) {
 					ray.alive = false;
 				}
 			}
+			norm_mask |= __ballot(ended_opaque);
 			n_samples += (uint32_t)__popcll(__ballot(have));
 		}
 		NGP_SECTION("other");
@@ -1006,6 +1028,7 @@
 	bitfield[i] = bits;
 }
 
+#ifdef NGP_ROUND_V1
 __global__ void coarse_occupancy_kernel(const uint8_t* __restrict__ bitfield, uint32_t* __restrict__ coarse) {
 	uint32_t w = blockIdx.x * blockDim.x + threadIdx.x;
 	if (w >= NERF_CASCADES * COARSE_WORDS_PER_MIP) return;
@@ -1027,6 +1050,39 @@
 	}
 	coarse[NERF_CASCADES * COARSE_WORDS_PER_MIP + w] = bits;
 }
+#else
+__global__ void coarse_occupancy_kernel(const uint8_t* __restrict__ bitfield, uint32_t* __restrict__ coarse) {
+	uint32_t w = blockIdx.x * blockDim.x + threadIdx.x;
+	if (w >= NERF_CASCADES * COARSE_WORDS_PER_MIP) return;
+	const uint32_t mip = w / COARSE_WORDS_PER_MIP, by = w & 31u, bz = (w >> 5) & 31u;
+	const uint2* src = (const uint2*)(bitfield + (size_t)(NERF_GRID_N_CELLS / 8) * mip);
+	uint2* words = (uint2*)(coarse + COARSE_SUMMARY_WORDS);
+	uint32_t bits = 0;
+	for (uint32_t bx = 0; bx < 32u; ++bx) {
+		const uint2 v = src[morton3D(bx, by, bz)];
+		const uint32_t block = occ_block4_of_block(bx, by, bz);
+		words[occ_block_word(mip, block)] = v;
+		bits |= ((v.x | v.y) != 0u ? 1u : 0u) << (block & 31u);
+	}
+	coarse[w] = bits;
+}
+__global__ void coarse16_occupancy_kernel(uint32_t* __restrict__ coarse) {
+	uint32_t w = threadIdx.x;
+	if (w >= NERF_CASCADES * 16) return;
+	const uint32_t mip = w / 16u;
+	uint32_t bits = 0;
+	for (uint32_t b = 0; b < 32u; ++b) {
+		const uint32_t b16 = (w & 15u) * 32u + b, x16 = b16 & 7u, y16 = (b16 >> 3) & 7u, z16 = b16 >> 6;
+		uint32_t any = 0;
+		for (uint32_t k = 0; k < 16u; ++k) {
+			const uint32_t block = occ_block4_of_block(x16 * 4u, y16 * 4u + (k & 3u), z16 * 4u + (k >> 2));
+			any |= (coarse[occ_summary4_word(mip, block)] >> (block & 31u)) & 0xfu;
+		}
+		bits |= (any != 0u ? 1u : 0u) << b;
+	}
+	coarse[NERF_CASCADES * COARSE_WORDS_PER_MIP + w] = bits;
+}
+#endif
 
 __global__ void bitfield_max_pool_kernel(uint32_t n_elements, const uint8_t* __restrict__ prev_level, uint8_t* __restrict__ next_level) {
 	uint32_t i = blockIdx.x * blockDim.x + threadIdx.x;
diff --git a/surface-irradiance-estimation-from-neural-radiance-fields_amd/csrc/ngp_kernels.h b/surface-irradiance-estimation-from-neural-radiance-fields_amd/csrc/ngp_kernels.h
--- a/surface-irradiance-estimation-from-neural-radiance-fields_amd/csrc/ngp_kernels.h
+++ b/surface-irradiance-estimation-from-neural-radiance-fields_amd/csrc/ngp_kernels.h
@@ -88,6 +88,12 @@
 	WideModel wide;
 };
 constexpr uint32_t COARSE_WORDS_PER_MIP = 32 * 32 * 32 / 32;
+constexpr uint32_t COARSE_SUMMARY_WORDS = NERF_CASCADES * COARSE_WORDS_PER_MIP + NERF_CASCADES * 16;
+#ifdef NGP_ROUND_V1
+constexpr uint32_t COARSE_TOTAL_WORDS = COARSE_SUMMARY_WORDS;
+#else
+constexpr uint32_t COARSE_TOTAL_WORDS = COARSE_SUMMARY_WORDS + NERF_CASCADES * (NERF_GRID_N_CELLS / 64) * 2;
+#endif
 
 struct CameraParams {
 	float m[12];
diff --git a/surface-irradiance-estimation-from-neural-radiance-fields_amd/csrc/ngp_model.cpp b/surface-irradiance-estimation-from-neural-radiance-fields_amd/csrc/ngp_model.cpp
--- a/surface-irradiance-estimation-from-neural-radiance-fields_amd/csrc/ngp_model.cpp
+++ b/surface-irradiance-estimation-from-neural-radiance-fields_amd/csrc/ngp_model.cpp
@@ -291,7 +291,7 @@
 	}
 	launch_density_grid_to_bitfield(ctx->d_density_f16.get(), (uint32_t)d.n_density_grid, max_cascade, ctx->d_density_f32.get(), ctx->d_partial.get(), ctx->d_bitfield.get(),
 	                                &ctx->bitfield_mean, ctx->stream);
-	ctx->d_coarse.reset((size_t)NERF_CASCADES * COARSE_WORDS_PER_MIP + NERF_CASCADES * 16);
+	ctx->d_coarse.reset((size_t)COARSE_TOTAL_WORDS);
 	launch_coarse_occupancy(ctx->d_bitfield.get(), ctx->d_coarse.get(), ctx->stream);
 	NGP_HIP_CHECK(hipStreamSynchronize(ctx->stream));
 	NGP_HIP_CHECK(hipGetLastError());
diff --git a/surface-irradiance-estimation-from-neural-radiance-fields_amd/csrc/ngp_multi.cpp b/surface-irradiance-estimation-from-neural-radiance-fields_amd/csrc/ngp_multi.cpp
--- a/surface-irradiance-estimation-from-neural-radiance-fields_amd/csrc/ngp_multi.cpp
+++ b/surface-irradiance-estimation-from-neural-radiance-fields_amd/csrc/ngp_multi.cpp
@@ -39,7 +39,7 @@
 	if (grid) {
 		const size_t n_cells = (size_t)NERF_GRID_N_CELLS * (primary->max_cascade + 1);
 		NGP_HIP_CHECK(hipMemcpyPeerAsync(peer->d_bitfield.get(), peer->device, primary->d_bitfield.get(), primary->device, (size_t)NERF_GRID_N_CELLS / 8 * NERF_CASCADES, s));
-		NGP_HIP_CHECK(hipMemcpyPeerAsync(peer->d_coarse.get(), peer->device, primary->d_coarse.get(), primary->device, ((size_t)NERF_CASCADES * COARSE_WORDS_PER_MIP + NERF_CASCADES * 16) * sizeof(uint32_t), s));
+		NGP_HIP_CHECK(hipMemcpyPeerAsync(peer->d_coarse.get(), peer->device, primary->d_coarse.get(), primary->device, (size_t)COARSE_TOTAL_WORDS * sizeof(uint32_t), s));
 		NGP_HIP_CHECK(hipMemcpyPeerAsync(peer->d_density_f32.get(), peer->device, primary->d_density_f32.get(), primary->device, n_cells * sizeof(float), s));
 		peer->bitfield_mean = primary->bitfield_mean;
 		peer->grid_rng_state = primary->grid_rng_state;
diff --git a/surface-irradiance-estimation-from-neural-radiance-fields_amd/csrc/occ_index.h b/surface-irradiance-estimation-from-neural-radiance-fields_amd/csrc/occ_index.h
--- /dev/null
+++ b/surface-irradiance-estimation-from-neural-radiance-fields_amd/csrc/occ_index.h
@@ -0,0 +1,42 @@
+#pragma once
+#include <stdint.h>
+
+#if defined(__HIPCC__) || defined(__CUDACC__)
+#define NGP_OCC_FN __host__ __device__ __forceinline__
+#else
+#define NGP_OCC_FN inline
+#endif
+
+namespace ngp {
+
+constexpr uint32_t OCC_GRIDSIZE = 128u;
+constexpr uint32_t OCC_BLOCKS_PER_MIP = (OCC_GRIDSIZE / 4u) * (OCC_GRIDSIZE / 4u) * (OCC_GRIDSIZE / 4u);
+constexpr uint32_t OCC_SUMMARY4_WORDS_PER_MIP = OCC_BLOCKS_PER_MIP / 32u;
+constexpr uint32_t OCC_SUMMARY16_WORDS_PER_MIP = 16u;
+
+NGP_OCC_FN uint32_t occ_expand_bits(uint32_t v) {
+	v = (v * 0x00010001u) & 0xFF0000FFu;
+	v = (v * 0x00000101u) & 0x0F00F00Fu;
+	v = (v * 0x00000011u) & 0xC30C30C3u;
+	v = (v * 0x00000005u) & 0x49249249u;
+	return v;
+}
+NGP_OCC_FN uint32_t occ_morton3D(uint32_t x, uint32_t y, uint32_t z) { return occ_expand_bits(x) | (occ_expand_bits(y) << 1) | (occ_expand_bits(z) << 2); }
+
+#ifdef NGP_ROUND_V1
+NGP_OCC_FN uint32_t occ_block4(uint32_t x, uint32_t y, uint32_t z) { return occ_morton3D(x >> 2, y >> 2, z >> 2); }
+NGP_OCC_FN uint32_t occ_block16(uint32_t x, uint32_t y, uint32_t z) { return occ_morton3D(x >> 4, y >> 4, z >> 4); }
+#else
+NGP_OCC_FN uint32_t occ_block4(uint32_t x, uint32_t y, uint32_t z) { return (x >> 2) | ((y >> 2) << 5) | ((z >> 2) << 10); }
+NGP_OCC_FN uint32_t occ_block16(uint32_t x, uint32_t y, uint32_t z) { return (x >> 4) | ((y >> 4) << 3) | ((z >> 4) << 6); }
+#endif
+NGP_OCC_FN uint32_t occ_block4_of_block(uint32_t bx, uint32_t by, uint32_t bz) { return occ_block4(bx << 2, by << 2, bz << 2); }
+NGP_OCC_FN uint32_t occ_block16_of_block(uint32_t bx, uint32_t by, uint32_t bz) { return occ_block16(bx << 2, by << 2, bz << 2); }
+NGP_OCC_FN uint32_t occ_bit_in_block(uint32_t x, uint32_t y, uint32_t z) {
+	return (x & 1u) | ((y & 1u) << 1) | ((z & 1u) << 2) | ((x & 2u) << 2) | ((y & 2u) << 3) | ((z & 2u) << 4);
+}
+NGP_OCC_FN uint32_t occ_block_word(uint32_t mip, uint32_t block) { return mip * OCC_BLOCKS_PER_MIP + block; }
+NGP_OCC_FN uint32_t occ_summary4_word(uint32_t mip, uint32_t block4) { return mip * OCC_SUMMARY4_WORDS_PER_MIP + (block4 >> 5); }
+NGP_OCC_FN uint32_t occ_summary16_word(uint32_t mip, uint32_t block16) { return mip * OCC_SUMMARY16_WORDS_PER_MIP + (block16 >> 5); }
+
+}
diff --git a/surface-irradiance-estimation-from-neural-radiance-fields_amd/csrc/wide_kernels.hip b/surface-irradiance-estimation-from-neural-radiance-fields_amd/csrc/wide_kernels.hip
--- a/surface-irradiance-estimation-from-neural-radiance-fields_amd/csrc/wide_kernels.hip
+++ b/surface-irradiance-estimation-from-neural-radiance-fields_amd/csrc/wide_kernels.hip
@@ -30,8 +30,8 @@
 	int iz = (int)(pos.z * (float)NERF_GRIDSIZE);
 	if (ix < 0 || ix >= (int)NERF_GRIDSIZE || iy < 0 || iy >= (int)NERF_GRIDSIZE || iz < 0 || iz >= (int)NERF_GRIDSIZE) return 1u;
 	const uint32_t idx = morton3D((uint32_t)ix, (uint32_t)iy, (uint32_t)iz);
-	const uint32_t b16 = idx >> 12;
-	if (!((s_coarse16[mip * 16u + (b16 >> 5)] >> (b16 & 31u)) & 1u)) return 16u;
+	const uint32_t b16 = occ_block16((uint32_t)ix, (uint32_t)iy, (uint32_t)iz);
+	if (!((s_coarse16[occ_summary16_word(mip, b16)] >> (b16 & 31u)) & 1u)) return 16u;
 	const uint32_t b4 = idx >> 6, key = (mip << 26) | b4;
 	if (cache.key != key) {
 		cache.bits = *(const uint2*)(bitfield + (size_t)b4 * 8 + (size_t)(NERF_GRID_N_CELLS / 8) * mip);
```

New measurement: 1131 Mrays/s, median of 6. 1.01x the previous value.
